# Fanchuana/OPUS-PLLM

Hardware: AMD Instinct MI355X
Metric: proteins_per_sec (higher is better)
Workload: dtype f16; 1 GPU; OPUS-PLLM-llama3_8b shape: batch 64/GPU, 512-residue proteins, 89-id prompt (+8 protein tokens = 96 positions), 32 new tokens, greedy (BASELINE configs[3] per-GPU shard: batch 512 over 8 GPUs); batch_per_gpu=64, residues=512, parallelism=replicas x1 (batch-sharded), all-gather of ids

## Files before the change

include/opus_pllm.h:

```cpp
#ifndef OPUS_PLLM_H
#define OPUS_PLLM_H

#include <stdint.h>

#ifdef __cplusplus
extern "C" {
#endif

#define OPUS_ABI_VERSION 10

enum opus_status {
    OPUS_OK = 0,
    OPUS_EBADARG = -1,
    OPUS_ESHAPE = -2,
    OPUS_EHIP = -3,
    OPUS_ERCCL = -4,
    OPUS_EUNSUPPORTED = -5,
    OPUS_ESTATE = -6
};

enum opus_dtype { OPUS_F16 = 0, OPUS_F32 = 1, OPUS_I32 = 2, OPUS_I64 = 3, OPUS_U8 = 4, OPUS_F8E4M3 = 5, OPUS_I8 = 6 };

typedef struct opus_config {
    int32_t enc_layers, enc_dim, enc_heads, enc_ffn, enc_vocab;
// ... 142 lines not shown
                                   int64_t n_slots, void *d_scratch, int64_t scratch_bytes, void *stream);

int opus_generate_lookup(opus_ctx *ctx, const void *d_embeds, const uint8_t *d_mask, int32_t B, int32_t T, int32_t max_new,
                         const int32_t *eos_ids, int32_t n_eos, int32_t pad_id, int32_t k, int32_t max_ngram, const int32_t *d_hist,
                         int32_t Lh, const int32_t *h_hist_len, int32_t *d_out_ids, int32_t *n_out, int64_t *stats, void *stream);
int opus_llama_verify_step(opus_ctx *ctx, const int32_t *d_tokens, int32_t n, const int32_t *d_draft_len, float *d_logits_all,
                           int32_t *d_argmax, int32_t *a, void *stream);
int opus_debug_lookup_draft(opus_ctx *ctx, const int32_t *d_hist, int32_t Lh, const int32_t *d_hist_len, int32_t R, int32_t k,
                            int32_t max_ngram, int32_t *d_draft, int32_t *d_draft_len, void *stream);
int opus_debug_last_qkv(opus_ctx *ctx, void *d_out, int32_t rows, void *stream);
int opus_debug_lookup_accept(opus_ctx *ctx, const int32_t *d_argmax, const int32_t *d_tokens, const int32_t *d_draft_len, int32_t R,
                             int32_t n, int32_t pre, int32_t *d_ids, int32_t stride, int32_t *d_fin, int32_t *d_step,
                             const int32_t *eos_ids, int32_t n_eos, int32_t pad_id, const int32_t *stop_ids, int32_t n_stop,
                             int32_t *d_next, int32_t *d_nunf, int32_t *h_words, void *stream);

int opus_debug_argmax_lse(opus_ctx *ctx, const float *d_logits, int32_t B, int32_t V, int32_t *d_idx, float *d_lse, void *stream);
int opus_debug_guidance(opus_ctx *ctx, float *d_logits, int32_t P, int32_t V, float guidance_scale, void *stream);

int opus_set_logits_processors(opus_ctx *ctx, float repetition_penalty, int32_t no_repeat_ngram_size, int32_t min_new_tokens,
                               const int32_t *bad_ids, const int32_t *bad_offsets, int32_t n_bad);
int opus_debug_logits_process(opus_ctx *ctx, float *d_logits, int32_t B, int32_t V, const int32_t *d_hist, int32_t hist_stride,
                              int32_t hist_len, const int32_t *eos_ids, int32_t n_eos, float repetition_penalty,
                              int32_t no_repeat_ngram_size, int32_t min_new_tokens, const int32_t *bad_ids,
                              const int32_t *bad_offsets, int32_t n_bad, void *stream);

int opus_set_token_constraint(opus_ctx *ctx, int32_t n_states, const int32_t *edge_off, const int32_t *edge_tok,
                              const int32_t *edge_next, int32_t n_edges, const uint8_t *completing, const int32_t *end_ids,
                              int32_t n_end, const int32_t *start, int32_t n_start, void *stream);
int opus_debug_token_constraint(opus_ctx *ctx, float *d_logits, int32_t B, int32_t V, const int32_t *d_hist, int32_t hist_stride,
                                int32_t hist_len, int32_t *d_state_out, void *stream);

int opus_debug_gemm(opus_ctx *ctx, const void *d_A, const void *d_W, const float *d_bias, const float *d_residual,
                    void *d_C, int32_t M, int32_t N, int32_t K, int32_t epi, int32_t out_f32, void *stream);
int opus_debug_gemm_norm(opus_ctx *ctx, const float *d_A, const void *d_W, void *d_C, int32_t M, int32_t N, int32_t K,
                         int32_t epi, int32_t out_f32, float eps, void *stream);
int opus_debug_gemm_slabs(opus_ctx *ctx, const void *d_A, const void *d_W, float *d_slabs, int32_t M, int32_t N, int32_t K,
                          int32_t *ks, void *stream);
int opus_debug_gemm_plan(opus_ctx *ctx, int32_t *plan);
int opus_debug_gemm_w8(opus_ctx *ctx, int32_t form, const void *d_A, const void *d_W, const void *d_q8, const void *d_e8,
                       const float *d_bias, const float *d_residual, void *d_C, int32_t M, int32_t N, int32_t K, int32_t epi,
                       int32_t out_f32, float eps, int32_t *ks, int32_t *ran_w8, void *stream);
int opus_debug_knob(opus_ctx *ctx, const char *name, int32_t value);
int opus_debug_gemm_rowscale(opus_ctx *ctx, const void *d_A, const void *d_W1, float *d_X, const void *d_W2, void *d_C,
                             int32_t M, int32_t N1, int32_t K1, int32_t N2, int32_t epi, float eps, int32_t *fused,
                             void *stream);
int opus_debug_gemm_rope(opus_ctx *ctx, const void *d_A, const void *d_W, const float *d_bias, void *d_out, int32_t M,
                         int32_t D, int32_t K, int32_t T, int32_t heads, int32_t allow_fuse, int32_t *fused, void *stream);
int opus_debug_gemm_ln(opus_ctx *ctx, const void *d_A, const void *d_W1, const float *d_b1, float *d_X, float *d_part, void *d_xh,
                       float *d_stat, const void *d_W2, const float *d_c2, const float *d_colsum, void *d_C, int32_t M, int32_t N1,
                       int32_t K1, int32_t N2, int32_t epi, int32_t rms, float eps, int32_t rope_T, const int32_t *d_rope_pos,
                       int32_t *produced, int32_t *plan, void *stream);
int opus_debug_attention(opus_ctx *ctx, const void *d_Q, const void *d_K, const void *d_V, void *d_O,
                         const int32_t *d_kstart, const int32_t *d_kend, int32_t B, int32_t T, int32_t heads,
                         int32_t group, int32_t head_dim, int32_t causal, float scale, void *stream);

int opus_debug_attn_prefill(opus_ctx *ctx, const void *d_Q, const void *d_K, const void *d_V, void *d_O, int64_t q_st, int64_t k_st,
                            int64_t v_st, int64_t o_st, int64_t q_sb, int64_t k_sb, int64_t v_sb, int64_t o_sb,
                            const int32_t *d_kstart, const int32_t *d_kend, const int32_t *d_cu, int32_t B, int32_t T,
                            int32_t heads, int32_t group, int32_t head_dim, int32_t causal, int32_t q_trim, float scale,
                            int32_t *qt_used, void *stream);

int opus_debug_attn_decode(opus_ctx *ctx, const void *d_qkv, const void *d_k_hist, const void *d_v_hist, const int32_t *d_kstart,
                           int32_t B, int32_t T0, int32_t step, void *d_out, void *d_k_new, void *d_v_new, void *stream);

int opus_debug_attn_decode_form(opus_ctx *ctx, const void *d_qkv, const float *d_slabs, int32_t ks, const float *d_row_ssq,
                                int32_t row_nblk, int32_t K, float eps, const float *d_bias, const void *d_k_hist,
                                const void *d_v_hist, const int32_t *d_kstart, int32_t B, int32_t T0, int32_t step,
                                int32_t out_tiled, void *d_out, void *d_k_new, void *d_v_new, void *d_k_cache, void *d_v_cache,
                                int32_t *gp_used, void *stream);

int opus_check_error(opus_ctx *ctx, void *stream);

int opus_beam_topk(opus_ctx *ctx, const float *d_run_scores, int32_t B, int32_t K, int32_t M, float *d_scores, int32_t *d_idx,
                   void *stream);
int opus_kv_reorder(opus_ctx *ctx, const int32_t *d_src_rows, int32_t R, void *stream);
int opus_beam_sample_topk(opus_ctx *ctx, const float *d_logits, const float *d_run_scores, int32_t B, int32_t K, int32_t M,
                          float temperature, float top_p, uint64_t seed, int32_t step, float *d_scores, int32_t *d_idx, void *stream);
int opus_set_sampling_top_k(opus_ctx *ctx, int32_t k);

int32_t opus_stream_lag(void);
int opus_stream_begin(opus_ctx *ctx, const void *d_embeds, const uint8_t *d_mask, int32_t B, int32_t T, int32_t max_new,
                      const int32_t *eos_ids, int32_t n_eos, int32_t pad_id, float temperature, float top_p, uint64_t seed,
                      int32_t *d_ids, void *stream);
int opus_stream_run(opus_ctx *ctx, int32_t t_min, int32_t min_free, int32_t t_max, int32_t *t_out, int32_t *h_end, void *stream);
int opus_stream_refill(opus_ctx *ctx, const opus_prefix_snap *snap, int32_t n, const int32_t *h_rows, const int32_t *h_src,
                       const float *d_last_logits, const int32_t *h_len, void *stream);
int opus_stream_end(opus_ctx *ctx, int32_t *h_end, void *stream);
int opus_debug_stream_state(opus_ctx *ctx, int32_t *h_kstart, int32_t *h_fin, int32_t *h_start, int32_t *h_end, int64_t *epoch,
                            int32_t poison, void *stream);

int opus_last_logits(opus_ctx *ctx, float *d_out, int32_t B, void *stream);

int64_t opus_stat(opus_ctx *ctx, const char *name);

int opus_timing_enable(opus_ctx *ctx, int32_t on);
int opus_timing_reset(opus_ctx *ctx);
int opus_timing_get(opus_ctx *ctx, const char *kernel_class, const char *phase, double *ms, int64_t *launches, double *bytes,
                    double *flops);
int opus_timing_names(char *buf, int32_t cap);

#ifdef __cplusplus
}
#endif
#endif
```

opus-pllm_amd/_cabi.py:

```python
from __future__ import annotations

import ctypes as C
import os
from typing import Optional

from .config import OpusConfig

_HERE = os.path.dirname(os.path.abspath(__file__))
BF16 = os.environ.get("OPUS_DTYPE", "fp16").lower() in ("bf16", "bfloat16")
LIB_PATH = os.environ.get("OPUS_LIB_PATH") or os.path.join(_HERE, "lib", "libopus_pllm_bf16.so" if BF16 else "libopus_pllm.so")
ABI_VERSION = 10

OPUS_F16, OPUS_F32, OPUS_I32, OPUS_I64, OPUS_U8 = 0, 1, 2, 3, 4
OPUS_F8E4M3, OPUS_I8 = 5, 6


def operand_dtype():
    import torch
    return torch.bfloat16 if BF16 else torch.float16


class OpusError(RuntimeError):
    def __init__(self, code: int, msg: str):
        super().__init__(f"libopus_pllm error {code}: {msg}")
# ... 65 lines not shown
    "opus_tile_weight": (C.c_int, [_P, _P, C.c_int64, C.c_int64, _P]),
    "opus_quantize_fp8": (C.c_int, [_P, C.c_int64, C.c_int64, _P, _P, _P, _P]),
    "opus_debug_gemm_w8": (C.c_int, [_P, C.c_int32, _P, _P, _P, _P, _P, _P, _P, C.c_int32, C.c_int32, C.c_int32, C.c_int32, C.c_int32,
                                     C.c_float, C.POINTER(C.c_int32), C.POINTER(C.c_int32), _P]),
    "opus_esm2_encode": (C.c_int, [_P, _P, _P, C.c_int32, C.c_int32, _P, _P]),
    "opus_esm2_encode_packed": (C.c_int, [_P, _P, C.POINTER(C.c_int32), C.c_int32, _P, _P]),
    "opus_esm2_last_hidden": (C.c_int, [_P, _P, C.c_int32, C.c_int32, _P]),
    "opus_projector_forward": (C.c_int, [_P, _P, C.c_int32, _P, _P, _P]),
    "opus_protein_projector": (C.c_int, [_P, _P, C.c_int32, _P, _P]),
    "opus_switch_projector": (C.c_int, [_P, _P, C.c_int32, _P, _P]),
    "opus_splice_pad": (C.c_int, [_P, _P, _P, C.c_int32, C.c_int32, _P, C.c_int32, C.c_int32, C.c_int32,
                                  _P, _P, _P, C.POINTER(C.c_int32), _P]),
    "opus_llama_prefill": (C.c_int, [_P, _P, _P, C.c_int32, C.c_int32, _P, _P]),
    "opus_llama_decode_step": (C.c_int, [_P, _P, _P, _P]),
    "opus_generate_greedy": (C.c_int, [_P, _P, _P, C.c_int32, C.c_int32, C.c_int32, C.POINTER(C.c_int32),
                                       C.c_int32, C.c_int32, _P, C.POINTER(C.c_int32), _P]),
    "opus_debug_gemm": (C.c_int, [_P, _P, _P, _P, _P, _P, C.c_int32, C.c_int32, C.c_int32, C.c_int32, C.c_int32, _P]),
    "opus_debug_gemm_norm": (C.c_int, [_P, _P, _P, _P, C.c_int32, C.c_int32, C.c_int32, C.c_int32, C.c_int32, C.c_float, _P]),
    "opus_debug_gemm_rope": (C.c_int, [_P, _P, _P, _P, _P, C.c_int32, C.c_int32, C.c_int32, C.c_int32, C.c_int32, C.c_int32, _P, _P]),
    "opus_debug_attention": (C.c_int, [_P, _P, _P, _P, _P, _P, _P, C.c_int32, C.c_int32, C.c_int32, C.c_int32,
                                       C.c_int32, C.c_int32, C.c_float, _P]),
    "opus_debug_attn_prefill": (C.c_int, [_P, _P, _P, _P, _P, C.c_int64, C.c_int64, C.c_int64, C.c_int64, C.c_int64, C.c_int64,
                                          C.c_int64, C.c_int64, _P, _P, _P, C.c_int32, C.c_int32, C.c_int32, C.c_int32, C.c_int32,
                                          C.c_int32, C.c_int32, C.c_float, C.POINTER(C.c_int32), _P]),
    "opus_generate_sample": (C.c_int, [_P, _P, _P, C.c_int32, C.c_int32, C.c_int32, C.POINTER(C.c_int32), C.c_int32, C.c_int32,
                                       C.c_float, C.c_float, C.c_uint64, _P, C.POINTER(C.c_int32), _P]),
    "opus_debug_sample": (C.c_int, [_P, _P, C.c_int32, C.c_float, C.c_float, C.c_uint64, C.c_int32, _P, _P]),
    "opus_timing_enable": (C.c_int, [_P, C.c_int32]),
    "opus_timing_reset": (C.c_int, [_P]),
    "opus_timing_get": (C.c_int, [_P, C.c_char_p, C.c_char_p, C.POINTER(C.c_double), C.POINTER(C.c_int64),
                                  C.POINTER(C.c_double), C.POINTER(C.c_double)]),
    "opus_timing_names": (C.c_int, [C.c_char_p, C.c_int32]),
    "opus_last_logits": (C.c_int, [_P, _P, C.c_int32, _P]),
    "opus_check_error": (C.c_int, [_P, _P]),
    "opus_beam_topk": (C.c_int, [_P, _P, C.c_int32, C.c_int32, C.c_int32, _P, _P, _P]),
    "opus_kv_reorder": (C.c_int, [_P, _P, C.c_int32, _P]),
    "opus_beam_sample_topk": (C.c_int, [_P, _P, _P, C.c_int32, C.c_int32, C.c_int32, C.c_float, C.c_float, C.c_uint64, C.c_int32,
                                        _P, _P, _P]),
    "opus_set_sampling_top_k": (C.c_int, [_P, C.c_int32]),
    "opus_set_stop_sequence": (C.c_int, [_P, C.POINTER(C.c_int32), C.c_int32]),
    "opus_debug_gemm_slabs": (C.c_int, [_P, _P, _P, _P, C.c_int32, C.c_int32, C.c_int32, C.POINTER(C.c_int32), _P]),
    "opus_debug_gemm_plan": (C.c_int, [_P, C.POINTER(C.c_int32)]),
    "opus_debug_knob": (C.c_int, [_P, C.c_char_p, C.c_int32]),
    "opus_stat": (C.c_int64, [_P, C.c_char_p]),
    "opus_debug_attn_decode": (C.c_int, [_P, _P, _P, _P, _P, C.c_int32, C.c_int32, C.c_int32, _P, _P, _P, _P]),
    "opus_debug_attn_decode_form": (C.c_int, [_P, _P, _P, C.c_int32, _P, C.c_int32, C.c_int32, C.c_float, _P, _P, _P, _P, C.c_int32,
                                              C.c_int32, C.c_int32, C.c_int32, _P, _P, _P, _P, _P, C.POINTER(C.c_int32), _P]),
    "opus_llama_forward": (C.c_int, [_P, _P, _P, C.c_int32, C.c_int32, _P, C.c_int32, _P, _P, _P, _P, C.c_int64, _P]),
    "opus_llama_forward_scratch_bytes": (C.c_int64, [C.POINTER(CConfig), C.c_int32, C.c_int32]),
    "opus_llama_prefix": (C.c_int, [_P, _P, _P, C.c_int32, C.c_int32, _P, _P, C.POINTER(C.c_int64), _P]),
    "opus_llama_score_continuations": (C.c_int, [_P, _P, C.c_int32, C.c_int32, _P, _P, _P, C.c_int32, C.c_int64, _P, _P, _P,
                                                 C.c_int64, _P]),
    "opus_llama_score_scratch_bytes": (C.c_int64, [C.POINTER(CConfig), C.c_int32, C.c_int32]),
    "opus_debug_attn_prefix": (C.c_int, [_P, _P, _P, _P, _P, C.c_int32, C.c_int32, C.c_int32, C.c_int32, _P, _P, _P]),
    "opus_llama_score_tree": (C.c_int, [_P, _P, C.c_int32, _P, _P, _P, C.c_int32, _P, C.c_int32, _P, _P, _P, C.c_int32, _P, _P, _P,
                                        C.c_int32, _P, C.c_int32, _P, _P, C.c_int32, C.c_int64, _P, _P, C.c_int64, _P, C.c_int64, _P]),
    "opus_llama_score_tree_scratch_bytes": (C.c_int64, [C.POINTER(CConfig), C.c_int32, C.c_int32, C.c_int32, C.c_int32, C.c_int32,
                                                        C.c_int32]),
    "opus_llama_dec_rows_cap": (C.c_int64, [C.POINTER(CConfig)]),
    "opus_llama_tree_max_depth": (C.c_int32, []),
    "opus_trie_path_sums": (C.c_int, [_P, _P, _P, _P, _P, _P, C.c_int32, C.c_int32, C.c_int32, _P, _P]),
    "opus_debug_attn_tree": (C.c_int, [_P, _P, _P, _P, _P, C.c_int32, C.c_int32, C.c_int32, _P, _P, _P, _P, _P]),
    "opus_debug_xent": (C.c_int, [_P, _P, C.c_int32, C.c_int32, _P, _P, _P, _P]),
    "opus_esm2_contacts_packed": (C.c_int, [_P, _P, C.POINTER(C.c_int32), C.c_int32, _P, _P, _P, C.c_int64, _P]),
    "opus_esm2_contacts_scratch_bytes": (C.c_int64, [C.POINTER(CConfig), C.POINTER(C.c_int32), C.c_int32]),
    "opus_debug_contacts": (C.c_int, [_P, _P, _P, C.c_int64, C.POINTER(C.c_int32), C.c_int32, C.c_int32, C.c_int32, _P, _P, _P, _P,
# ... 53 lines not shown
```

opus-pllm_amd/csrc/api.cpp:

```cpp
#include "../../include/opus_pllm.h"
#include "common.h"

#include <cmath>
#include <cstdarg>
#include <cstdio>
#include <cstdlib>
#include <cstring>
#include <algorithm>
#include <atomic>
#include <map>
#include <string>
#include <vector>

using namespace opus;

static thread_local char g_err[512] = "";
static int fail(int code, const char *fmt, ...) {
    va_list ap;
    va_start(ap, fmt);
    vsnprintf(g_err, sizeof(g_err), fmt, ap);
    va_end(ap);
    return code;
}
#define HIPC(expr)                                                                                   \
// ... 15 lines not shown
};

struct EncLayer {
    const float *bqkv, *bo, *b1, *b2, *sqkv, *s1;
    const half_t *wqkv, *wo, *w1, *w2;
};
struct DecLayer {
    const half_t *wqkv = nullptr, *wo = nullptr, *wgu = nullptr, *wd = nullptr;
    const float *bqkv = nullptr;
    const uint8_t *q8_qkv = nullptr, *q8_o = nullptr, *q8_gu = nullptr, *q8_d = nullptr;
    const int8_t *e8_qkv = nullptr, *e8_o = nullptr, *e8_gu = nullptr, *e8_d = nullptr;
    const half_t *w1 = nullptr, *w2 = nullptr;
    const float *bo = nullptr, *b1 = nullptr, *b2 = nullptr, *ln1w = nullptr, *ln1b = nullptr, *ln2w = nullptr, *ln2b = nullptr;
};

struct TimeRec {
    int klass, phase;
    hipEvent_t e0, e1;
    double bytes, flops;
};

struct StepPlan {
    int rows = -1;
    bool guided = false;
    int stride = -1;
    int32_t *ids = nullptr;
    int n_eos = -1, pad = 0;
    float temp = 0.f, top_p = 1.f;
    int top_k = 0, n_stop = 0;
    int outs = 0;
    bool lproc = false;
    bool cons = false;
    int budget = -1;
};
static bool same_step(const StepPlan &a, const StepPlan &b) {
    return a.rows == b.rows && a.guided == b.guided && a.stride == b.stride && a.ids == b.ids && a.n_eos == b.n_eos && a.pad == b.pad &&
           a.temp == b.temp && a.top_p == b.top_p && a.top_k == b.top_k && a.n_stop == b.n_stop && a.outs == b.outs &&
           a.lproc == b.lproc && a.cons == b.cons && a.budget == b.budget;
}

struct opus_ctx {
    opus_config cfg;
    int device = 0;
    std::map<std::string, Tensor> w;
    bool resolved = false;
    const half_t *enc_emb = nullptr, *dec_emb = nullptr, *lm_head = nullptr, *proj_w = nullptr, *dec_pos = nullptr;
    const float *enc_lnfw = nullptr, *enc_lnfb = nullptr, *proj_b = nullptr, *dec_lnfw = nullptr, *dec_lnfb = nullptr;
    std::vector<EncLayer> enc;
    std::vector<DecLayer> dec;
    std::vector<const half_t *> sw_w;
    std::vector<const float *> sw_b;
    char *ws = nullptr;
    size_t ws_bytes = 0;
    float *e_x, *e_hid, *p_pool_dummy, *e_part, *e_stat;
    int32_t *e_cu, *e_pos;
    std::vector<int32_t> h_cu;
    int64_t enc_rows = 0;
    half_t *e_xn, *e_qkv, *e_ctx, *e_h1;
    half_t *p_xn, *p_y, *p_z[2];
    float *d_x, *d_xl, *d_logits, *d_pval, *gemm_ws, *d_probs, *d_zpart, *d_spart, *d_part, *d_stat;
    int32_t *d_cand_i, *d_cand_n;
    uint64_t *d_seed;
    int32_t *d_chosen;
    int samp_top_k = 0;
    float *d_bthr = nullptr, *d_blse = nullptr;
    int64_t gemm_ws_bytes = 0;
    half_t *d_xn, *d_qkv, *d_ctx, *d_act, *d_xln, *kc, *vc;
    float *cs_enc, *cs_dec, *cs_row;
    int32_t *d_kstart, *d_step, *d_next, *d_fin, *d_nunf, *d_eos, *d_plan, *d_pidx, *d_stop, *d_cnt;
    int n_stop = 0;
    static constexpr int POLL_RING = 4, POLL_LAG = 2;
    int32_t *h_nunf = nullptr;
    hipEvent_t poll_ev[POLL_RING] = {nullptr, nullptr, nullptr, nullptr};
    int64_t cache_sl, cache_sb, cache_sh;
    int cur_B = 0, cur_T = 0;
    bool prefilled = false;
    struct GraphEntry {
        hipGraphExec_t exec = nullptr;
        StepPlan key;
        uint64_t used = 0;
    };
    static constexpr int MAX_GRAPHS = 4;
    std::vector<GraphEntry> graphs;
    uint64_t graph_clock = 0;
    int64_t graph_instantiations = 0;
    int64_t graph_replays = 0;
    int64_t decode_steps = 0;
    char *gen_mem = nullptr;
    GenOutDesc *d_gen = nullptr;
    GenOutDesc h_gen{};
    float *d_gpsum = nullptr, *d_gthr = nullptr;
    bool lproc_on = false;
    LogitsProcDesc h_lproc{1.0f, 0, 0, 0, {}, {}};
    char *lproc_mem = nullptr;
    LogitsProcDesc *d_lproc = nullptr;
    int32_t *d_lstep = nullptr, *d_ridx = nullptr;
    GenOutDesc *d_gen_raw = nullptr, *d_gen_proc = nullptr;
    float *d_rlse = nullptr, *d_rawh = nullptr;
    bool cons_on = false;
    char *cons_tab = nullptr, *cons_mem = nullptr;
    size_t cons_tab_bytes = 0;
    TokenConstraintDesc *d_cons = nullptr;
    int32_t *d_cstate = nullptr, *d_cstep = nullptr;
    int32_t cons_n_start = 0, cons_max_id = -1;
    int32_t cons_start_div = 1;
    char *guid_mem = nullptr;
    float *d_gscale = nullptr, *d_gdpsum = nullptr, *d_gmax = nullptr, *d_glog = nullptr, *d_glse = nullptr, *guid_keep = nullptr;
    int gemm_w8 = 0;
    int64_t w8_gemms = 0;
    int gemm_plan[GEMM_PLAN_WORDS] = {-1, -1, -1, -1, -1, -1, -1, -1};
    float *d_ssq = nullptr;
    int64_t ssq_cap = 0;
    bool timing = false;
    int phase = PH_OTHER;
    std::vector<TimeRec> recs;
    int proj_rows = 0;
    char *proj_big = nullptr;
    half_t *kv_tmp = nullptr;
    int64_t epoch = 0;
    std::vector<int32_t> h_kstart;
    int32_t *behind_tbl = nullptr;
// ... 210 lines not shown
    HIPC(hipMemset(c->kc, 0, (size_t)c->cache_sl * cfg->dec_layers * sizeof(half_t)));
    HIPC(hipMemset(c->vc, 0, (size_t)c->cache_sl * cfg->dec_layers * sizeof(half_t)));
    HIPC(hipHostMalloc((void **)&c->h_nunf, ((size_t)cfg->max_new_tokens + 4) * sizeof(int32_t), hipHostMallocDefault));
    for (auto &e : c->poll_ev) HIPC(hipEventCreateWithFlags(&e, hipEventDisableTiming));
    *out = c;
    return OPUS_OK;
}

static void timing_clear(opus_ctx *c) {
    for (auto &r : c->recs) {
        (void)hipEventDestroy(r.e0);
        (void)hipEventDestroy(r.e1);
    }
    c->recs.clear();
}

static void drop_graphs(opus_ctx *c) {
    for (auto &g : c->graphs)
        if (g.exec) (void)hipGraphExecDestroy(g.exec);
    c->graphs.clear();
    if (c->stream_graph.exec) (void)hipGraphExecDestroy(c->stream_graph.exec);
    c->stream_graph = opus_ctx::GraphEntry();
}

extern "C" int opus_ctx_destroy(opus_ctx *c) {
    if (!c) return OPUS_OK;
    (void)hipSetDevice(c->device);
    timing_clear(c);
    drop_graphs(c);
    if (c->ws) (void)hipFree(c->ws);
    if (c->proj_big) (void)hipFree(c->proj_big);
    if (c->kv_tmp) (void)hipFree(c->kv_tmp);
    if (c->gen_mem) (void)hipFree(c->gen_mem);
    if (c->lproc_mem) (void)hipFree(c->lproc_mem);
    if (c->cons_tab) (void)hipFree(c->cons_tab);
    if (c->cons_mem) (void)hipFree(c->cons_mem);
    if (c->guid_mem) (void)hipFree(c->guid_mem);
    if (c->guid_keep) (void)hipFree(c->guid_keep);
    if (c->behind_tbl) (void)hipFree(c->behind_tbl);
    if (c->h_nunf) (void)hipHostFree(c->h_nunf);
    if (c->stream_mem) (void)hipFree(c->stream_mem);
    if (c->h_poll) (void)hipHostFree(c->h_poll);
    if (c->lk_mem) (void)hipFree(c->lk_mem);
    if (c->h_lk) (void)hipHostFree(c->h_lk);
    for (auto &e : c->poll_ev) if (e) (void)hipEventDestroy(e);
    delete c;
    return OPUS_OK;
}

extern "C" int opus_bind_weight(opus_ctx *c, const char *name, const void *d_ptr, int dtype, int ndim,
                                const int64_t *shape) {
    if (!c || !name || !d_ptr || !shape) return fail(OPUS_EBADARG, "null argument");
    if (ndim < 1 || ndim > 4) return fail(OPUS_EBADARG, "ndim %d", ndim);
    const size_t nlen = strlen(name);
    const bool is_q8 = nlen > 3 && !strcmp(name + nlen - 3, ".q8"), is_e8 = nlen > 3 && !strcmp(name + nlen - 3, ".e8");
    if (is_q8 ? dtype != OPUS_F8E4M3 : is_e8 ? dtype != OPUS_I8 : (dtype != OPUS_F16 && dtype != OPUS_F32))
        return fail(OPUS_EBADARG, "weights are fp16 or fp32 (FP8 panels '*.q8': e4m3, their row exponents '*.e8': int8)");
    if (((uintptr_t)d_ptr) & 15) return fail(OPUS_EBADARG, "%s: pointer must be 16-byte aligned", name);
    Tensor t;
    t.p = d_ptr;
    t.dtype = dtype;
    t.shape.assign(shape, shape + ndim);
    c->w[name] = t;
    c->resolved = false;
    drop_graphs(c);
    return OPUS_OK;
// ... 119 lines not shown
        if (!c->timing) return;
        tl_launch_ev = nullptr;
        if (ev.main_used) {
            c->recs.push_back(TimeRec{ev.main_class >= 0 ? ev.main_class : klass, c->phase, ev.main0, ev.main1, bytes, flops});
            (void)hipEventDestroy(b0); (void)hipEventDestroy(b1);
        } else {
            (void)hipEventRecord(b1, s);
            c->recs.push_back(TimeRec{klass, c->phase, b0, b1, bytes, flops});
            (void)hipEventDestroy(ev.main0); (void)hipEventDestroy(ev.main1);
        }
        if (ev.aux_used) c->recs.push_back(TimeRec{KC_REDUCE, c->phase, ev.aux0, ev.aux1, ev.aux_bytes, 0.0});
        else { (void)hipEventDestroy(ev.aux0); (void)hipEventDestroy(ev.aux1); }
    }
};

struct GemmAsk {
    half_t *xh = nullptr;
    int xh_tiled = 0;
    bool rs_on = false;
    float rs_eps = 0.f;
    int rs_nblk = 0;
    const float *rope_cs = nullptr;
    const int32_t *rope_pos = nullptr;
    int rope_T = 0, rope_cols = 0, rope_qcols = 0;
    float rope_qscale = 1.0f;
    float *ln_part = nullptr;
    half_t *ln_xh = nullptr;
    const float *ln_stat = nullptr, *ln_colsum = nullptr;
    int force_wide = 0, slab_only = 0;
    int a_tiled = 0, c_tiled = 0;
    int *pp_plan = nullptr;
    const uint8_t *q8 = nullptr;
    const int8_t *e8 = nullptr;
    GemmAsk &copy16(half_t *dst, bool tiled = false) { xh = dst; xh_tiled = dst && tiled; return *this; }
    GemmAsk &scale_rows(float eps, int nblk) { rs_on = true; rs_eps = eps; rs_nblk = nblk; return *this; }
    GemmAsk &rope(const float *cs, const int32_t *pos, int T, int D, float qscale) {
        if (cs) { rope_cs = cs; rope_pos = pos; rope_T = T; rope_cols = 2 * D; rope_qcols = D; rope_qscale = qscale; }
        return *this;
    }
    GemmAsk &ln_produce(float *part, half_t *x16) { if (part) { ln_part = part; ln_xh = x16; } return *this; }
    GemmAsk &ln_consume(const float *stat, const float *colsum) { if (stat) { ln_stat = stat; ln_colsum = colsum; } return *this; }
    GemmAsk &slabs() { force_wide = slab_only = 1; return *this; }
    GemmAsk &tiled_a(int on) { a_tiled = on; return *this; }
    GemmAsk &tiled_c(int on) { c_tiled = on; return *this; }
    GemmAsk &report_pp(int *plan) { pp_plan = plan; return *this; }
    GemmAsk &w8(const uint8_t *q, const int8_t *e) { if (q && e) { q8 = q; e8 = e; } return *this; }
};
struct GemmGot {
    int xh_done = 0, rope_done = 0, ln_done = 0, ks = 1, ssq_nblk = 0;
};

static int gemm_any(opus_ctx *c, hipStream_t s, const half_t *A, const float *Af, float eps, int64_t lda, const half_t *W,
                    int M, int N, int K, const float *bias, int epi, const float *residual, void *C, int64_t ldc,
                    int out_f32, const GemmAsk &ask = GemmAsk(), GemmGot *got = nullptr) {
    GemmGot mine;
    if (!got) got = &mine;
    *got = GemmGot();
    GemmParams p;
    p.A = A; p.Af = Af; p.norm_eps = eps; p.lda = lda; p.W = W; p.M = M; p.N = N; p.K = K; p.bias = bias;
    p.residual = residual; p.ldr = ldc; p.C = C; p.ldc = ldc; p.out_f32 = out_f32; p.epi = epi;
    p.ws = c->gemm_ws; p.ws_bytes = c->gemm_ws_bytes;
    p.xh_out = ask.xh; p.ssq_out = c->d_ssq; p.fused_done = &got->xh_done; p.ssq_cap = c->ssq_cap; p.nblk_out = &got->ssq_nblk;
    p.rope_cs = ask.rope_cs; p.rope_T = ask.rope_T; p.rope_cols = ask.rope_cols; p.rope_qcols = ask.rope_qcols;
    p.rope_qscale = ask.rope_qscale; p.rope_done = &got->rope_done; p.rope_pos = ask.rope_pos;
    p.row_ssq = nullptr; p.row_nblk = 0;
    if (ask.rs_on) { p.row_ssq = c->d_ssq; p.row_nblk = ask.rs_nblk; p.norm_eps = ask.rs_eps; }
    p.force_wide = ask.force_wide; p.slab_only = ask.slab_only; p.ks_out = &got->ks;
    if (ask.ln_part) { p.xh_out = ask.ln_xh; p.ssq_out = nullptr; p.ln_part = ask.ln_part; p.ln_done = &got->ln_done; }
    if (ask.ln_stat) { p.ln_stat = ask.ln_stat; p.ln_colsum = ask.ln_colsum; }
    p.combine_cnt = c->d_cnt;
    p.pp_plan = ask.pp_plan;
    for (int i = 0; i < GEMM_PLAN_WORDS; ++i) c->gemm_plan[i] = -1;
    p.plan = c->gemm_plan;
    c->gemm_w8 = 0;
    p.q8 = ask.q8; p.e8 = ask.e8; p.ran_w8 = &c->gemm_w8;
    p.a_tiled = ask.a_tiled; p.xh_tiled = ask.xh_tiled; p.c_tiled = ask.c_tiled;
    const int nout = epi == EPI_SILU_GU16 ? N / 2 : N;
    const double bytes = 2.0 * N * K + (Af ? 4.0 : 2.0) * M * K + (double)M * nout * (out_f32 ? 4 : 2) +
                         (residual ? 4.0 * M * nout : 0.0);
    int klass = M <= SKINNY_MAX_M ? KC_SKINNY : KC_TILE;
    hipError_t e;
    {
        Timed t(c, s, klass, bytes, 2.0 * M * N * (double)K);
        e = launch_gemm(p, s, &klass);
    }
    if (e != hipSuccess) return fail(OPUS_EHIP, "gemm M=%d N=%d K=%d failed: %s", M, N, K, hipGetErrorString(e));
    c->w8_gemms += c->gemm_w8;
    return OPUS_OK;
}
static int gemm(opus_ctx *c, hipStream_t s, const half_t *A, int64_t lda, const half_t *W, int M, int N, int K,
                const float *bias, int epi, const float *residual, void *C, int64_t ldc, int out_f32,
                const GemmAsk &ask = GemmAsk(), GemmGot *got = nullptr) {
    return gemm_any(c, s, A, nullptr, 0.f, lda, W, M, N, K, bias, epi, residual, C, ldc, out_f32, ask, got);
}
struct ResidShadow {
    const float *xh_src = nullptr;
    int ssq_nblk = 0;
    bool xln_tiled = false;
    void produced(const float *x, const GemmGot &got, bool tiled = false) {
        xh_src = got.xh_done ? x : nullptr;
        if (got.xh_done) ssq_nblk = got.ssq_nblk;
        xln_tiled = got.xh_done && tiled;
    }
};
static bool fuse_rows() {
    static const bool off = getenv("OPUS_NO_ROW_FUSION") != nullptr;
    return !off;
}
#define KLF(klass, bytes, flops, call)                                                                \
    do {                                                                                              \
        hipError_t e_;                                                                                \
        {                                                                                             \
            Timed t_(c, s, klass, bytes, flops);                                                      \
            e_ = (call);                                                                              \
        }                                                                                             \
        if (e_ != hipSuccess) return fail(OPUS_EHIP, "%s failed: %s", #call, hipGetErrorString(e_)); \
    } while (0)
#define KL(klass, bytes, call) KLF(klass, bytes, 0.0, call)

// ... 435 lines not shown
        const int n = B - r0 < c->proj_rows ? B - r0 : c->proj_rows;
        OPC(protein_projector_rows(c, s, d_pooled + r0 * din, n, c->p_y));
        if (d_proj_out)
            HIPC(hipMemcpyAsync((half_t *)d_proj_out + r0 * dmid, c->p_y, (size_t)n * dmid * sizeof(half_t), hipMemcpyDeviceToDevice, s));
        OPC(switch_projector_rows(c, s, c->p_y, n, (half_t *)d_out + r0 * SW));
    }
    return OPUS_OK;
}

extern "C" int opus_splice_pad(opus_ctx *c, const int64_t *d_ids, const uint8_t *d_mask, int32_t B, int32_t Tt,
                               const void *d_prot, int32_t n_prot, int32_t inference_mode, int32_t max_length,
                               void *d_embeds, uint8_t *d_mask_out, int32_t *d_pos_out, int32_t *T_out, void *stream) {
    OPC(need_ready(c));
    if (!d_ids || !d_prot || !d_embeds || !d_mask_out || !d_pos_out || !T_out) return fail(OPUS_EBADARG, "splice_pad: null pointer");
    const opus_config &g = c->cfg;
    if (B < 1 || B > g.max_batch || Tt < 1) return fail(OPUS_ESHAPE, "splice_pad: B=%d T_text=%d out of range", B, Tt);
    hipStream_t s = (hipStream_t)stream;
    c->phase = PH_SPLICE;
    KL(KC_OTHER, 9.0 * B * Tt, launch_splice_plan(d_ids, d_mask, B, Tt, g.n_prot_tokens, max_length, g.dec_vocab, c->d_plan, s));
    int32_t tail[3];
    HIPC(hipMemcpyAsync(tail, c->d_plan + 4 * B, sizeof(tail), hipMemcpyDeviceToHost, s));
    HIPC(hipStreamSynchronize(s));
    if (tail[2]) return fail(OPUS_EBADARG, "splice_pad: token id outside [0, vocab) (and not -200)");
    if (tail[1] > n_prot) return fail(OPUS_ESHAPE, "splice_pad: rows consume %d protein blocks, %d supplied", tail[1], n_prot);
    if (tail[0] > g.max_prompt) return fail(OPUS_ESHAPE, "splice_pad: spliced length %d exceeds max_prompt=%d", tail[0], g.max_prompt);
    if (tail[0] < 1) return fail(OPUS_ESHAPE, "splice_pad: every row is empty");
    *T_out = tail[0];
    KL(KC_OTHER, 2.0 * B * tail[0] * g.dec_dim * 2,
       launch_splice_fill(d_ids, d_mask, B, Tt, (const half_t *)d_prot, g.n_prot_tokens, g.dec_dim, g.dec_vocab, c->dec_emb,
                          c->d_plan, tail[0], inference_mode ? 1 : 0, (half_t *)d_embeds, d_mask_out, d_pos_out, s));
    return OPUS_OK;
}

static int lm_head(opus_ctx *c, hipStream_t s, ResidShadow &sh, int B, float *out = nullptr) {
    const opus_config &g = c->cfg;
    return gemm_norm(c, s, sh, c->d_xl, g.dec_rms_eps, c->d_xln, c->lm_head, B, g.dec_vocab, g.dec_dim, EPI_NONE, out ? out : c->d_logits,
                     g.dec_vocab, 1);
}

static int fanout_rows(opus_ctx *c, hipStream_t s, int B, int nret) {
    const opus_config &g = c->cfg;
    KL(KC_OTHER, 4.0 * (B + B * nret) * g.dec_vocab, launch_row_fanout(c->d_probs, c->d_logits, g.dec_vocab, B, nret, c->d_kstart, s));
    return OPUS_OK;
}


static int reset_step(opus_ctx *c, hipStream_t s, int T0, int step = 0) {
    const int32_t v[2] = {step, T0};
    HIPC(launch_upload_i32(v, 2, c->d_step, s));
    return OPUS_OK;
}

template <class Head>
static int finish_prefill(opus_ctx *c, hipStream_t s, int B, int T, int nret, bool have_last, Head head) {
    const int H = c->cfg.dec_dim;
    if (!have_last) KL(KC_OTHER, 8.0 * B * H, launch_take_last(c->d_x, B, T, H, c->d_xl, s));
    OPC(head(nret > 1 ? c->d_probs : nullptr));
    if (nret > 1) OPC(fanout_rows(c, s, B, nret));
    OPC(reset_step(c, s, T));
    c->cur_B = B * nret;
    c->cur_T = T;
    c->prefilled = true;
    return OPUS_OK;
}

static int attn_decode(opus_ctx *c, hipStream_t s, const ResidShadow &sh, int l, int B, int T, int slab_ks = 0, const float *bias = nullptr,
                       int out_tiled = 0) {
    const opus_config &g = c->cfg;
    AttnDecodeParams a;
    a.qkv = c->d_qkv; a.slabs = nullptr; a.ks = 0; a.slab_stride = 0; a.row_ssq = nullptr; a.row_nblk = 0; a.eps = 0.f; a.K = 0;
// ... 41 lines not shown
    a.q_sb = a.k_sb = a.v_sb = (int64_t)T * QKV;
    a.q_st = a.k_st = a.v_st = QKV;
    a.O = c->d_ctx; a.o_sb = (int64_t)T * QD; a.o_st = QD;
    a.kstart = c->d_kstart; a.kend = nullptr;
    a.B = B; a.T = T; a.heads = nh; a.group = nh / nkv; a.head_dim = hd; a.causal = 1;
    a.scale = 1.0f / sqrtf((float)hd);
    KLF(KC_ATTN_PREFILL, 2.0 * M * (QKV + QD), 2.0 * B * (double)T * T * QD, launch_attn_prefill(a, s));
    return OPUS_OK;
}

static int opt_layer(opus_ctx *c, hipStream_t s, const DecLayer &L, int l, float *x, half_t *xn, int M, int B, int T, bool decode,
                     const ContRows *cont = nullptr, int nret = 1) {
    const opus_config &g = c->cfg;
    const int H = g.dec_dim, F = g.dec_ffn;
    const int QKV = (g.dec_heads + 2 * g.dec_kv_heads) * g.dec_head_dim, QD = g.dec_heads * g.dec_head_dim;
    KL(KC_NORM, 6.0 * M * H, launch_layernorm(x, L.ln1w, L.ln1b, g.dec_rms_eps, M, H, xn, nullptr, s));
    OPC(gemm(c, s, xn, H, L.wqkv, M, QKV, H, L.bqkv, EPI_NONE, nullptr, c->d_qkv, QKV, 0));
    if (decode) OPC(attn_decode(c, s, ResidShadow(), l, B, T));
    else OPC(attn_prefill(c, s, l, B, T, cont, nret));
    OPC(gemm(c, s, c->d_ctx, QD, L.wo, M, H, QD, L.bo, EPI_NONE, x, x, H, 1));
    KL(KC_NORM, 6.0 * M * H, launch_layernorm(x, L.ln2w, L.ln2b, g.dec_rms_eps, M, H, xn, nullptr, s));
    if (g.dec_act == 0) {
        OPC(gemm(c, s, xn, H, L.w1, M, F, H, L.b1, EPI_GELU, nullptr, c->d_act, F, 0));
    } else {
        OPC(gemm(c, s, xn, H, L.w1, M, F, H, L.b1, EPI_NONE, nullptr, c->d_act, F, 0));
        KL(KC_OTHER, 4.0 * M * F, launch_relu_h(c->d_act, (int64_t)M * F, s));
    }
    OPC(gemm(c, s, c->d_act, F, L.w2, M, H, F, L.b2, EPI_NONE, x, x, H, 1));
    return OPUS_OK;
}

static int lm_head_opt(opus_ctx *c, hipStream_t s, int B, float *out = nullptr) {
    const opus_config &g = c->cfg;
    KL(KC_NORM, 6.0 * B * g.dec_dim, launch_layernorm(c->d_xl, c->dec_lnfw, c->dec_lnfb, g.dec_rms_eps, B, g.dec_dim, c->d_xln, nullptr, s));
    return gemm(c, s, c->d_xln, g.dec_dim, c->lm_head, B, g.dec_vocab, g.dec_dim, nullptr, EPI_NONE, nullptr, out ? out : c->d_logits,
                g.dec_vocab, 1);
}

static int prefill_opt(opus_ctx *c, hipStream_t s, const half_t *embeds, const uint8_t *mask, int B, int T, bool all_rows,
                       const ContRows *cont, int nret) {
    const opus_config &g = c->cfg;
    const int H = g.dec_dim, M = B * T;
    HIPC(hipMemsetAsync(c->d_cnt, 0, HANDOFF_ERR * sizeof(int32_t), s));
    if (!cont) KL(KC_OTHER, 1.0 * M, launch_mask_to_kstart(mask, B, T, c->d_kstart, s));
    KL(KC_OTHER, 6.0 * M * H, launch_h2f(embeds, c->d_x, (int64_t)M * H, s));
    KL(KC_OTHER, 10.0 * M * H, launch_add_pos(c->d_x, c->dec_pos, cont ? cont->nkst : c->d_kstart, nullptr, 0, B, T, H, g.dec_max_pos + 1, s));
    for (int l = 0; l < g.dec_layers; ++l) OPC(opt_layer(c, s, c->dec[l], l, c->d_x, c->d_xn, M, B, T, false, cont, nret));
    if (all_rows) return OPUS_OK;
    return finish_prefill(c, s, B, T, nret, false, [&](float *out) { return lm_head_opt(c, s, B, out); });
}

static int decode_step_opt(opus_ctx *c, hipStream_t s) {
    const opus_config &g = c->cfg;
    const int B = c->cur_B, T = c->cur_T, H = g.dec_dim;
    KL(KC_OTHER, 10.0 * B * H, launch_add_pos(c->d_xl, c->dec_pos, c->d_kstart, c->d_step, -1, B, 1, H, g.dec_max_pos + 1, s));
    for (int l = 0; l < g.dec_layers; ++l) OPC(opt_layer(c, s, c->dec[l], l, c->d_xl, c->d_xln, B, B, T, true));
    OPC(lm_head_opt(c, s, B));
    KL(KC_OTHER, 8.0, launch_step_advance(c->d_step, s));
    return OPUS_OK;
}

static int prefill(opus_ctx *c, hipStream_t s, const half_t *embeds, const uint8_t *mask, int B, int T, bool all_rows = false,
                   const ContRows *cont = nullptr, int nret = 1) {
    c->phase = cont && !cont->app_lens ? PH_SCORE : PH_PREFILL;
    if (cont && cont->w8) c->phase = PH_DECODE;
    if (cont) {
        all_rows = true;
    } else {
        new_epoch(c);
        if (all_rows) {
            c->prefilled = false;
            c->cur_B = 0;
        }
    }
    if (c->cfg.dec_arch == 1) return prefill_opt(c, s, embeds, mask, B, T, all_rows, cont, nret);
    const opus_config &g = c->cfg;
    const int H = g.dec_dim, F = g.dec_ffn, nh = g.dec_heads, nkv = g.dec_kv_heads, hd = g.dec_head_dim;
    const int QKV = (nh + 2 * nkv) * hd, QD = nh * hd;
    const int M = B * T;
    HIPC(hipMemsetAsync(c->d_cnt, 0, HANDOFF_ERR * sizeof(int32_t), s));
    if (!cont) KL(KC_OTHER, 1.0 * M, launch_mask_to_kstart(mask, B, T, c->d_kstart, s));
    KL(KC_OTHER, 6.0 * M * H, launch_h2f(embeds, c->d_x, (int64_t)M * H, s));
    static const bool no_ln_env = getenv("OPUS_NO_LN_FUSION") != nullptr;
    const bool no_ln_fusion = no_ln_env || g_knobs.no_ln_fusion;
    const bool qkv_pp = !no_ln_fusion && (H & 255) == 0 && (QKV & 255) == 0 && gemm_goes_pp(M, QKV);
    const bool gu_pp = !no_ln_fusion && (H & 255) == 0 && (F & 127) == 0 && gemm_goes_pp(M, 2 * F);
    bool have_stat = false, last_rows_done = false;
    auto finalize = [&]() -> int {
        KL(KC_NORM, 8.0 * M * (H / 64) + 8.0 * M, launch_ln_finalize(c->d_part, M, H / 64, H, g.dec_rms_eps, 1, c->d_stat, s));
        return OPUS_OK;
    };
    ResidShadow sh;
    GemmGot got;
    const bool w8 = cont && cont->w8;
    auto ask8 = [&](GemmAsk a, const uint8_t *q, const int8_t *e) { return w8 ? a.w8(q, e) : a; };
    for (int l = 0; l < g.dec_layers; ++l) {
// ... 7 lines not shown
        OPC(attn_prefill(c, s, l, B, T, cont, nret));
        if (l + 1 == g.dec_layers && T > 1 && !all_rows && !g_knobs.misc[7]) {
            half_t *ctx_last = c->d_qkv;
            KL(KC_OTHER, 4.0 * B * QD, launch_take_last(reinterpret_cast<const float *>(c->d_ctx), B, T, QD / 2, reinterpret_cast<float *>(ctx_last), s));
            KL(KC_OTHER, 8.0 * B * H, launch_take_last(c->d_x, B, T, H, c->d_xl, s));
            const GemmAsk copy_xl = GemmAsk().copy16(fuse_rows() && B <= 96 ? c->d_xln : nullptr);
            OPC(gemm(c, s, ctx_last, QD, L.wo, B, H, QD, nullptr, EPI_NONE, c->d_xl, c->d_xl, H, 1, copy_xl, &got));
            sh.produced(c->d_xl, got);
            OPC(gemm_norm(c, s, sh, c->d_xl, g.dec_rms_eps, c->d_xln, L.wgu, B, 2 * F, H, EPI_SILU_GU16, c->d_act, F, 0));
            OPC(gemm(c, s, c->d_act, F, L.wd, B, H, F, nullptr, EPI_NONE, c->d_xl, c->d_xl, H, 1, copy_xl, &got));
            sh.produced(c->d_xl, got);
            last_rows_done = true;
            break;
        }
        GemmAsk wo;
        if (gu_pp) wo.ln_produce(c->d_part, c->d_xn);
        else if (fuse_rows() && M <= 96) wo.copy16(c->d_xn);
        OPC(gemm(c, s, c->d_ctx, QD, L.wo, M, H, QD, nullptr, EPI_NONE, c->d_x, c->d_x, H, 1, ask8(wo, L.q8_o, L.e8_o), &got));
        sh.produced(c->d_x, got);
        have_stat = got.ln_done != 0;
        if (have_stat) {
            OPC(finalize());
            OPC(gemm(c, s, c->d_xn, H, L.wgu, M, 2 * F, H, nullptr, EPI_SILU_GU16, nullptr, c->d_act, F, 0, GemmAsk().ln_consume(c->d_stat, nullptr)));
        } else {
            OPC(gemm_norm(c, s, sh, c->d_x, g.dec_rms_eps, c->d_xn, L.wgu, M, 2 * F, H, EPI_SILU_GU16, c->d_act, F, 0, nullptr,
                          ask8(GemmAsk(), L.q8_gu, L.e8_gu)));
        }
        const bool next_pp = qkv_pp && l + 1 < g.dec_layers;
        OPC(gemm(c, s, c->d_act, F, L.wd, M, H, F, nullptr, EPI_NONE, c->d_x, c->d_x, H, 1, ask8(GemmAsk().ln_produce(next_pp ? c->d_part : nullptr, c->d_xn), L.q8_d, L.e8_d), &got));
        have_stat = got.ln_done != 0;
        if (have_stat) OPC(finalize());
    }
    if (all_rows) return OPUS_OK;
    return finish_prefill(c, s, B, T, nret, last_rows_done, [&](float *out) { return lm_head(c, s, sh, B, out); });
}

static int decode_step(opus_ctx *c, hipStream_t s, const int32_t *d_tok) {
    c->phase = PH_DECODE;
    const opus_config &g = c->cfg;
    const int B = c->cur_B, T = c->cur_T;
    const int H = g.dec_dim, F = g.dec_ffn, nh = g.dec_heads, nkv = g.dec_kv_heads, hd = g.dec_head_dim;
    const int QKV = (nh + 2 * nkv) * hd, QD = nh * hd;
    const int ctx_cap = g.max_prompt + g.max_new_tokens;
    const bool rowscale = g.dec_arch == 0 && fuse_rows() && B > SKINNY_MAX_M && B <= MID_MAX_M && (H & 255) == 0;
    const bool qkv_tiled = rowscale && gemm_stream_would(B, QKV, H, 1, 1, 1, c->gemm_ws_bytes);
    const bool wo_tiled = rowscale && gemm_stream_would(B, H, QD, 0, 1, 0, c->gemm_ws_bytes);
    const bool down_tiled = rowscale && (F & 63) == 0 && gemm_stream_would(B, H, F, 0, 1, 0, c->gemm_ws_bytes);
    KL(KC_OTHER, 6.0 * B * H, launch_embed_tokens(d_tok, c->dec_emb, B, H, g.dec_vocab, c->d_xl, rowscale ? c->d_xln : nullptr,
                                                  rowscale ? c->d_ssq : nullptr, qkv_tiled ? 1 : 0, c->cs_dec, c->d_kstart, c->d_step, -1,
                                                  hd / 2, c->cs_row, c->d_cnt, HANDOFF_ERR, s));
    if (g.dec_arch == 1) return decode_step_opt(c, s);
    ResidShadow sh;
    if (rowscale) { sh.xh_src = c->d_xl; sh.ssq_nblk = H >> 8; sh.xln_tiled = qkv_tiled; }
    GemmGot got;
    half_t *const copy_xl = fuse_rows() && B <= 96 ? c->d_xln : nullptr;
    for (int l = 0; l < g.dec_layers; ++l) {
        const DecLayer &L = c->dec[l];
        if (rowscale && sh.xh_src == c->d_xl) {
            sh.xh_src = nullptr;
            OPC(gemm(c, s, c->d_xln, H, L.wqkv, B, QKV, H, L.bqkv, EPI_NONE, nullptr, c->d_qkv, QKV, 0,
                     GemmAsk().slabs().scale_rows(g.dec_rms_eps, sh.ssq_nblk).tiled_a(sh.xln_tiled).w8(L.q8_qkv, L.e8_qkv), &got));
            OPC(attn_decode(c, s, sh, l, B, T, got.ks > 1 ? got.ks : 0, L.bqkv, wo_tiled ? 1 : 0));
        } else {
            OPC(gemm_norm(c, s, sh, c->d_xl, g.dec_rms_eps, c->d_xln, L.wqkv, B, QKV, H, EPI_NONE, c->d_qkv, QKV, 0, L.bqkv,
                          GemmAsk().w8(L.q8_qkv, L.e8_qkv)));
            OPC(attn_decode(c, s, sh, l, B, T, 0, nullptr, wo_tiled ? 1 : 0));
        }
        OPC(gemm(c, s, c->d_ctx, QD, L.wo, B, H, QD, nullptr, EPI_NONE, c->d_xl, c->d_xl, H, 1, GemmAsk().copy16(copy_xl).tiled_a(wo_tiled).w8(L.q8_o, L.e8_o), &got));
        sh.produced(c->d_xl, got);
        const bool act_tiled = down_tiled && sh.xh_src == c->d_xl && gemm_goes_wide(B, 2 * F);
        OPC(gemm_norm(c, s, sh, c->d_xl, g.dec_rms_eps, c->d_xln, L.wgu, B, 2 * F, H, EPI_SILU_GU16, c->d_act, F, 0, nullptr, GemmAsk().tiled_c(act_tiled).w8(L.q8_gu, L.e8_gu)));
        const bool next_tiled = qkv_tiled && l + 1 < g.dec_layers;
        OPC(gemm(c, s, c->d_act, F, L.wd, B, H, F, nullptr, EPI_NONE, c->d_xl, c->d_xl, H, 1, GemmAsk().copy16(copy_xl, next_tiled).tiled_a(act_tiled).w8(L.q8_d, L.e8_d), &got));
        sh.produced(c->d_xl, got, next_tiled);
    }
    OPC(lm_head(c, s, sh, B));
    KL(KC_OTHER, 8.0, launch_step_advance(c->d_step, s));
    return OPUS_OK;
}

static int handoff_check(opus_ctx *c, hipStream_t s) {
    int32_t err = 0;
    HIPC(hipMemcpyAsync(&err, c->d_cnt + HANDOFF_ERR, sizeof(err), hipMemcpyDeviceToHost, s));
    HIPC(hipStreamSynchronize(s));
    if (!err) return OPUS_OK;
    HIPC(hipMemsetAsync(c->d_cnt, 0, HANDOFF_WORDS * sizeof(int32_t), s));
    return fail(OPUS_EHIP, "an in-launch hand-off (split-K combine) gave up waiting for its partner: results of this call are invalid");
}

extern "C" int opus_check_error(opus_ctx *c, void *stream) {
    if (!c) return fail(OPUS_EBADARG, "ctx is null");
    HIPC(hipSetDevice(c->device));
    return handoff_check(c, (hipStream_t)stream);
}

static int check_prefill_args(opus_ctx *c, const void *e, const uint8_t *m, int B, int T) {
    if (!e || !m) return fail(OPUS_EBADARG, "prefill: null pointer");
    if (B < 1 || B > c->cfg.max_batch || T < 1 || T > c->cfg.max_prompt)
        return fail(OPUS_ESHAPE, "prefill: B=%d T=%d exceed capacity (%d, %d)", B, T, c->cfg.max_batch, c->cfg.max_prompt);
    return OPUS_OK;
}

extern "C" int opus_llama_prefill(opus_ctx *c, const void *d_embeds, const uint8_t *d_mask, int32_t B, int32_t T,
                                  float *d_last_logits, void *stream) {
    OPC(need_ready(c));
    OPC(check_prefill_args(c, d_embeds, d_mask, B, T));
    hipStream_t s = (hipStream_t)stream;
    OPC(prefill(c, s, (const half_t *)d_embeds, d_mask, B, T));
    if (d_last_logits)
// ... 693 lines not shown
    if (P < 1 || M < 1 || ld_nodes < 2) return fail(OPUS_ESHAPE, "trie_path_sums: P=%d M=%d nodes=%d", P, M, ld_nodes);
    HIPC(hipSetDevice(c->device));
    hipStream_t s = (hipStream_t)stream;
    c->phase = PH_SCORE;
    KL(KC_OTHER, 12.0 * P * M, launch_tree_path_sums(d_node_lp, d_trie, d_par, d_depth, d_member_node, P, M, ld_nodes, d_member_lp, s));
    return OPUS_OK;
}

extern "C" int opus_debug_attn_tree(opus_ctx *c, const void *d_qkv, const void *d_k_hist, const void *d_v_hist, const int32_t *d_kstart,
                                    int32_t P, int32_t Tp, int32_t R, const int32_t *h_src, const int32_t *h_par, const int32_t *h_depth,
                                    void *d_out, void *stream) {
    if (!c || !d_qkv || !d_k_hist || !d_v_hist || !d_kstart || !h_src || !h_par || !h_depth || !d_out)
        return fail(OPUS_EBADARG, "debug_attn_tree: null pointer");
    const opus_config &g = c->cfg;
    if (P < 1 || P > g.max_batch || Tp < 1 || Tp > g.max_prompt || R < 1)
        return fail(OPUS_ESHAPE, "debug_attn_tree: P=%d Tp=%d R=%d exceed the context (%d, %d)", P, Tp, R, g.max_batch, g.max_prompt);
    OPC(check_tree_rows("debug_attn_tree", R, P, h_src, h_par, h_depth));
    return debug_attn_prefix_run(c, "debug_attn_tree", d_qkv, d_k_hist, d_v_hist, d_kstart, P, Tp, R, 1, h_src, h_par, d_out, stream);
}

enum { GEN_LOGPROBS = 1, GEN_SCORES = 2, GEN_LOGITS = 4 };

static int ensure_gen_mem(opus_ctx *c) {
    if (c->gen_mem) return OPUS_OK;
    const size_t B = c->cfg.max_batch;
    const size_t o_ps = align_up(sizeof(GenOutDesc)), o_thr = o_ps + align_up(APART * B * sizeof(float));
    HIPC(hipMalloc((void **)&c->gen_mem, o_thr + align_up(B * sizeof(float))));
    c->d_gen = reinterpret_cast<GenOutDesc *>(c->gen_mem);
    c->d_gpsum = reinterpret_cast<float *>(c->gen_mem + o_ps);
    c->d_gthr = reinterpret_cast<float *>(c->gen_mem + o_thr);
    return OPUS_OK;
}

static int ensure_lproc_mem(opus_ctx *c) {
    if (c->lproc_mem) return OPUS_OK;
    const size_t B = c->cfg.max_batch, N = c->cfg.max_new_tokens;
    const size_t o_st = align_up(sizeof(LogitsProcDesc)), o_gr = o_st + align_up(B * sizeof(int32_t)),
                 o_gp = o_gr + align_up(sizeof(GenOutDesc)), o_ls = o_gp + align_up(sizeof(GenOutDesc)),
                 o_rh = o_ls + align_up(B * sizeof(float));
    HIPC(hipMalloc((void **)&c->lproc_mem, o_rh + align_up(B * N * sizeof(float))));
    c->d_lproc = reinterpret_cast<LogitsProcDesc *>(c->lproc_mem);
    c->d_ridx = reinterpret_cast<int32_t *>(c->lproc_mem + o_st);
    c->d_lstep = c->d_ridx;
    c->d_gen_raw = reinterpret_cast<GenOutDesc *>(c->lproc_mem + o_gr);
    c->d_gen_proc = reinterpret_cast<GenOutDesc *>(c->lproc_mem + o_gp);
    c->d_rlse = reinterpret_cast<float *>(c->lproc_mem + o_ls);
    c->d_rawh = reinterpret_cast<float *>(c->lproc_mem + o_rh);
    return OPUS_OK;
}

static int ensure_guid_mem(opus_ctx *c, bool keep) {
    const size_t B = c->cfg.max_batch;
    if (!c->guid_mem) {
        const size_t rows = align_up(2 * B * sizeof(float));
        const size_t o_ps = align_up(sizeof(float)), o_mx = o_ps + align_up(APART * B * sizeof(float)), o_lg = o_mx + rows,
                     o_ls = o_lg + rows;
        HIPC(hipMalloc((void **)&c->guid_mem, o_ls + rows));
        c->d_gscale = reinterpret_cast<float *>(c->guid_mem);
        c->d_gdpsum = reinterpret_cast<float *>(c->guid_mem + o_ps);
        c->d_gmax = reinterpret_cast<float *>(c->guid_mem + o_mx);
        c->d_glog = reinterpret_cast<float *>(c->guid_mem + o_lg);
        c->d_glse = reinterpret_cast<float *>(c->guid_mem + o_ls);
    }
    if (keep && !c->guid_keep) HIPC(hipMalloc((void **)&c->guid_keep, align_up((B / 2) * (size_t)c->cfg.dec_vocab * sizeof(float))));
    return OPUS_OK;
}
// ... 3 lines not shown
    memcpy(&w, &g, sizeof(w));
    HIPC(launch_upload_i32(&w, 1, reinterpret_cast<int32_t *>(c->d_gscale), s));
    return OPUS_OK;
}

static int upload_lproc(opus_ctx *c, const LogitsProcDesc &h, hipStream_t s) {
    const int32_t *w = reinterpret_cast<const int32_t *>(&h);
    const int head = (int)(offsetof(LogitsProcDesc, bad_off) / sizeof(int32_t)) + h.n_bad + 1;
    int32_t *dw = reinterpret_cast<int32_t *>(c->d_lproc);
    HIPC(launch_upload_i32(w, head, dw, s));
    const int n_ids = h.bad_off[h.n_bad];
    const int o_ids = (int)(offsetof(LogitsProcDesc, bad_ids) / sizeof(int32_t));
    if (n_ids) HIPC(launch_upload_i32(w + o_ids, n_ids, dw + o_ids, s));
    return OPUS_OK;
}

static int upload_gen_desc(const GenOutDesc &h, GenOutDesc *d, hipStream_t s) {
    HIPC(launch_upload_i32(reinterpret_cast<const int32_t *>(&h), (int)(sizeof(GenOutDesc) / sizeof(int32_t)),
                           reinterpret_cast<int32_t *>(d), s));
    return OPUS_OK;
}

static int select_next(opus_ctx *c, hipStream_t s, const StepPlan &p) {
    const int max_new = p.stride, n_eos = p.n_eos, pad_id = p.pad;
    int32_t *d_out = p.ids;
    c->phase = PH_DECODE;
    const opus_config &g = c->cfg;
    const int32_t *chosen = nullptr;
    const bool guid = p.guided;
    const int HB = guid ? p.rows / 2 : p.rows;
    const bool proc = p.lproc || p.cons || guid;
    const bool lp = p.outs & GEN_LOGPROBS, sc = p.outs & (GEN_SCORES | GEN_LOGITS);
    const size_t BV = (size_t)HB * g.dec_vocab;
    if (proc) {
        if (p.outs & GEN_LOGITS)
            KL(KC_OTHER, 8.0 * BV, launch_gen_scores(c->d_logits, HB, g.dec_vocab, c->d_gen_raw, c->d_step, max_new, 0.f, 1.f,
                                                     nullptr, nullptr, s));
        if (guid) {
            KL(KC_GUIDANCE, 8.0 * BV, launch_guidance_lse_partial(c->d_logits, 2 * HB, g.dec_vocab, c->d_pval, c->d_gdpsum, s));
            KL(KC_GUIDANCE, 1024.0 * HB, launch_guidance_lse_final(c->d_pval, c->d_gdpsum, 2 * HB, c->d_gmax, c->d_glog, c->d_glse, s));
            KL(KC_GUIDANCE, (lp ? 16.0 : 12.0) * BV,
               launch_guidance_combine(c->d_logits, c->d_logits + BV, HB, g.dec_vocab, c->d_gmax, c->d_glog, c->d_gmax + HB,
                                       c->d_glog + HB, c->d_gscale, lp ? c->guid_keep : nullptr, s));
        } else if (lp) {
            KL(KC_OTHER, 4.0 * BV, launch_argmax_lse_partial(c->d_logits, HB, g.dec_vocab, c->d_pval, c->d_pidx, c->d_gpsum, s));
            KL(KC_OTHER, 512.0 * HB, launch_argmax_lse_final(c->d_pval, c->d_pidx, c->d_gpsum, HB, c->d_ridx, c->d_rlse, s));
        }
        if (p.lproc)
            KL(KC_LOGITPROC, 12.0 * HB * max_new,
               launch_logits_proc(c->d_logits, HB, g.dec_vocab, d_out, max_new, c->d_step, max_new, c->d_eos, n_eos, c->d_lproc,
                                  lp && !guid ? c->d_rawh : nullptr, s));
        if (p.cons)
            KL(KC_CONSTRAINT, 4.0 * BV,
               launch_token_constraint(c->d_logits, HB, g.dec_vocab, d_out, max_new, c->d_step, max_new, c->d_cons, s));
    }
    if (p.temp > 0.f) {
        KL(KC_OTHER, 4.0 * 4 * HB * g.dec_vocab,
           launch_sample_select(c->d_logits, HB, g.dec_vocab, p.temp, p.top_p, p.top_k, c->d_seed, c->d_step,
                                c->d_pval, c->d_pidx, c->d_probs, c->d_cand_i, c->d_cand_n, c->d_zpart, c->d_spart, c->d_chosen, nullptr,
                                lp && !proc ? c->d_gpsum : nullptr, sc ? c->d_gthr : nullptr, s));
        chosen = c->d_chosen;
    } else if (lp && !proc) {
        KL(KC_OTHER, 4.0 * HB * g.dec_vocab,
           launch_argmax_lse_partial(c->d_logits, HB, g.dec_vocab, c->d_pval, c->d_pidx, c->d_gpsum, s));
    } else {
        KL(KC_OTHER, 4.0 * HB * g.dec_vocab, launch_argmax_partial(c->d_logits, HB, g.dec_vocab, c->d_pval, c->d_pidx, s));
    }
    if (proc ? (p.outs & GEN_SCORES) != 0 : sc)
        KL(KC_OTHER, 4.0 * HB * g.dec_vocab * (1 + ((p.outs & GEN_SCORES) ? 1 : 0) + ((p.outs & GEN_LOGITS) && !proc ? 1 : 0)),
           launch_gen_scores(c->d_logits, HB, g.dec_vocab, proc ? c->d_gen_proc : c->d_gen, c->d_step, max_new, p.temp,
                             p.top_p, c->d_pval, p.temp > 0.f ? c->d_gthr : nullptr, s));
    if (lp && proc)
        KL(KC_OTHER, 512.0 * HB + 8.0 * HB * max_new,
           launch_argmax_rawlp_step(c->d_pval, c->d_pidx, guid ? c->d_glse : c->d_rlse, p.lproc && !guid ? c->d_rawh : nullptr, chosen, HB, c->d_eos, n_eos, pad_id, c->d_fin, d_out,
                                    max_new, c->d_step, c->d_next, c->d_nunf, c->d_stop, p.n_stop, guid ? c->guid_keep : c->d_logits,
                                    g.dec_vocab, c->d_gen_proc, s));
    else if (lp)
        KL(KC_OTHER, 512.0 * HB + 8.0 * HB,
           launch_argmax_lse_step(c->d_pval, c->d_pidx, c->d_gpsum, chosen, HB, c->d_eos, n_eos, pad_id, c->d_fin, d_out, max_new,
                                  c->d_step, c->d_next, c->d_nunf, c->d_stop, p.n_stop, c->d_logits, g.dec_vocab, c->d_gen, s));
    else
        KL(KC_OTHER, 512.0 * HB,
           launch_argmax_step(c->d_pval, c->d_pidx, chosen, HB, c->d_eos, n_eos, pad_id, c->d_fin, d_out, max_new, c->d_step,
                              c->d_next, c->d_nunf, c->d_stop, p.n_stop, s));
    if (guid) KL(KC_GUIDANCE, 8.0 * HB, launch_guidance_pair_next(c->d_next, HB, s));
    return OPUS_OK;
}

static int greedy_body(opus_ctx *c, hipStream_t s, const StepPlan &p) {
    OPC(select_next(c, s, p));
    return decode_step(c, s, c->d_next);
}

static int capture_step(opus_ctx *c, hipStream_t s, int (*body)(opus_ctx *, hipStream_t, const StepPlan &), const StepPlan &p,
                        hipGraphExec_t *exec) {
    hipGraph_t graph = nullptr;
    HIPC(hipStreamBeginCapture(s, hipStreamCaptureModeThreadLocal));
    int rc = body(c, s, p);
    hipError_t ee = hipStreamEndCapture(s, &graph);
    if (rc != OPUS_OK) { if (graph) (void)hipGraphDestroy(graph); return rc; }
    if (ee != hipSuccess) return fail(OPUS_EHIP, "hipStreamEndCapture: %s", hipGetErrorString(ee));
    ee = hipGraphInstantiate(exec, graph, nullptr, nullptr, 0);
    (void)hipGraphDestroy(graph);
    if (ee != hipSuccess) { *exec = nullptr; return fail(OPUS_EHIP, "hipGraphInstantiate: %s", hipGetErrorString(ee)); }
    ++c->graph_instantiations;
    return OPUS_OK;
}

static int begin_generation(opus_ctx *c, const char *who, float temperature, float top_p, int32_t max_new, const int32_t *eos_ids,
                            int32_t n_eos, const uint64_t *seed, int rows, int steps, hipStream_t s) {
    if (temperature < 0.f || top_p <= 0.f || top_p > 1.f) return fail(OPUS_EBADARG, "%s: temperature >= 0 and 0 < top_p <= 1", who);
    if (max_new < 1 || max_new > c->cfg.max_new_tokens)
        return fail(OPUS_ESHAPE, "%s: max_new=%d exceeds max_new_tokens=%d", who, max_new, c->cfg.max_new_tokens);
    if (n_eos < 0 || n_eos > 64 || (n_eos > 0 && !eos_ids)) return fail(OPUS_EBADARG, "%s: eos list", who);
    if (n_eos) HIPC(hipMemcpyAsync(c->d_eos, eos_ids, n_eos * sizeof(int32_t), hipMemcpyHostToDevice, s));
    HIPC(hipMemcpyAsync(c->d_seed, seed, sizeof(*seed), hipMemcpyHostToDevice, s));
    HIPC(hipMemsetAsync(c->d_fin, 0, rows * sizeof(int32_t), s));
    HIPC(hipMemsetAsync(c->d_nunf, 0, (size_t)steps * sizeof(int32_t), s));
    return OPUS_OK;
}

static int set_cons_start_div(opus_ctx *c, int32_t div, hipStream_t s) {
    if (div == c->cons_start_div) return OPUS_OK;
    int32_t *w = reinterpret_cast<int32_t *>(c->d_cons) + offsetof(TokenConstraintDesc, start_div) / sizeof(int32_t);
    HIPC(launch_upload_i32(&div, 1, w, s));
    c->cons_start_div = div;
    return OPUS_OK;
}

static int generate_impl(opus_ctx *c, const void *d_embeds, const uint8_t *d_mask, int32_t B, int32_t T, int32_t max_new,
                         const int32_t *eos_ids, int32_t n_eos, int32_t pad_id, float temperature, float top_p, uint64_t seed,
                         int32_t *d_out_ids, int32_t *n_out, void *stream, const GenOutDesc *outs = nullptr, int32_t nret = 1,
                         const BehindArgs *behind = nullptr, const float *guidance = nullptr) {
    OPC(need_ready(c));
    if (!behind) OPC(check_prefill_args(c, d_embeds, d_mask, B, T));
    else if (B < 1 || B > c->cfg.max_batch) return fail(OPUS_ESHAPE, "generate: B=%d decoder rows, the context holds max_batch=%d", B, c->cfg.max_batch);
    OPC(check_fanout(c, B, nret, "generate"));
    const int32_t BN = B * nret;
    if (!d_out_ids || !n_out) return fail(OPUS_EBADARG, "generate_greedy: null pointer");
    hipStream_t s = (hipStream_t)stream;
    const opus_config &g = c->cfg;
    OPC(begin_generation(c, "generate_greedy", temperature, top_p, max_new, eos_ids, n_eos, &seed, BN, max_new, s));
    StepPlan plan;
    plan.rows = BN; plan.guided = guidance != nullptr; plan.stride = max_new; plan.ids = d_out_ids; plan.n_eos = n_eos; plan.pad = pad_id;
    plan.temp = temperature; plan.top_p = top_p; plan.top_k = c->samp_top_k; plan.n_stop = c->n_stop;
    plan.lproc = c->lproc_on; plan.cons = c->cons_on;
    if (outs) plan.outs = (outs->token_lp ? GEN_LOGPROBS : 0) | (outs->scores ? GEN_SCORES : 0) | (outs->logits ? GEN_LOGITS : 0);
    if (plan.outs) {
        OPC(ensure_gen_mem(c));
        c->h_gen = *outs;
        HIPC(hipMemcpyAsync(c->d_gen, &c->h_gen, sizeof(GenOutDesc), hipMemcpyHostToDevice, s));
    }
    const int32_t HB = guidance ? B / 2 : B;
    if (c->cons_on && c->cons_n_start != 1 && c->cons_n_start != HB)
        return fail(OPUS_ESHAPE, "generate: the token constraint has %d per-row start states, the batch %d rows", c->cons_n_start, HB);
    if (c->cons_on) OPC(set_cons_start_div(c, nret, s));
    if (guidance) {
        OPC(ensure_guid_mem(c, plan.outs & GEN_LOGPROBS));
        OPC(upload_guidance_scale(c, *guidance, s));
    }
    if (c->lproc_on || c->cons_on || guidance) {
        if (c->lproc_on && max_new > LP_MAX_HIST)
            return fail(OPUS_ESHAPE, "generate: logits processors keep a history of at most %d ids (max_new=%d)", LP_MAX_HIST, max_new);
        OPC(ensure_lproc_mem(c));
        if (c->lproc_on) OPC(upload_lproc(c, c->h_lproc, s));
        if (plan.outs) {
            OPC(upload_gen_desc(GenOutDesc{nullptr, nullptr, outs->logits, nullptr}, c->d_gen_raw, s));
            OPC(upload_gen_desc(GenOutDesc{outs->token_lp, outs->scores, nullptr, nullptr}, c->d_gen_proc, s));
        }
    }
    if (behind) OPC(prefill_behind(c, s, *behind, (const half_t *)d_embeds, B, T));
    else OPC(prefill(c, s, (const half_t *)d_embeds, d_mask, B, T, false, nullptr, nret));

    const bool use_graph = s != nullptr && !c->timing && !getenv("OPUS_NO_GRAPH");
    opus_ctx::GraphEntry *ge = nullptr;
    if (use_graph)
        for (auto &e : c->graphs)
            if (e.exec && same_step(e.key, plan)) { ge = &e; break; }
    const bool same_graph = ge != nullptr;
    std::vector<int32_t> nunf(max_new, 1);
    int produced = 0;
    for (int i = 0; i < max_new; ++i) {
        if (i + 1 == max_new) {
            OPC(select_next(c, s, plan));
            produced = i + 1;
            break;
        }
        ++c->decode_steps;
        if (!use_graph || (i == 0 && !same_graph)) {
            OPC(greedy_body(c, s, plan));
        } else {
            if (!ge) {
                opus_ctx::GraphEntry e;
                OPC(capture_step(c, s, greedy_body, plan, &e.exec));
                e.key = plan;
                if ((int)c->graphs.size() >= opus_ctx::MAX_GRAPHS) {
                    size_t v = 0;
                    for (size_t k = 1; k < c->graphs.size(); ++k) if (c->graphs[k].used < c->graphs[v].used) v = k;
                    (void)hipGraphExecDestroy(c->graphs[v].exec);
                    c->graphs.erase(c->graphs.begin() + v);
                }
                c->graphs.push_back(e);
                ge = &c->graphs.back();
            }
            ge->used = ++c->graph_clock;
// ... 499 lines not shown
    c->lk_kstart.assign((size_t)c->cur_B, 0);
    HIPC(hipMemcpyAsync(c->lk_kstart.data(), c->d_kstart, (size_t)c->cur_B * sizeof(int32_t), hipMemcpyDeviceToHost, s));
    HIPC(hipStreamSynchronize(s));
    c->lk_epoch = c->epoch;
    return OPUS_OK;
}

static int verify_pass(opus_ctx *c, hipStream_t s, const int32_t *x, int ld_x, int n, int Tp) {
    const opus_config &g = c->cfg;
    const int R = c->cur_B, M = R * n, H = g.dec_dim, V = g.dec_vocab, G = g.dec_heads / g.dec_kv_heads;
    if (!c->behind_tbl) HIPC(hipMalloc((void **)&c->behind_tbl, (size_t)behind_table_words(g) * sizeof(int32_t)));
    std::vector<int32_t> src((size_t)R);
    for (int r = 0; r < R; ++r) src[r] = r;
    PrefixTables t;
    build_prefix_tables(g, c->lk_kstart, Tp, src.data(), R, n, t);
    if (t.nblocks > attn_prefix_max_blocks(R, g.max_batch, G, n)) return fail(OPUS_EHIP, "verify pass: block table overflow");
    const int o_lens = (int)t.w.size();
    t.w.insert(t.w.end(), (size_t)R, n);
    if ((int64_t)t.w.size() > behind_table_words(g)) return fail(OPUS_EHIP, "verify pass: table overflow");
    int32_t *tbl = c->behind_tbl;
    c->phase = PH_DECODE;
    HIPC(launch_upload_i32(t.w.data(), (int)t.w.size(), tbl, s));
    KL(KC_OTHER, 4.0 * M * H, launch_lookup_embed(x, ld_x, R, n, c->dec_emb, H, V, c->d_xn, s));
    ContRows cr;
    cr.nkst = tbl + t.nkst;
    cr.nblocks = t.nblocks;
    cr.attn = prefix_params(c, tbl, t, Tp, n, c->d_qkv, nullptr, nullptr, c->d_ctx);
    cr.app_lens = tbl + o_lens;
    cr.w8 = true;
    OPC(prefill(c, s, c->d_xn, nullptr, R, n, true, &cr));
    c->phase = PH_DECODE;
    if (g.dec_arch == 1) {
        KL(KC_NORM, 6.0 * M * H, launch_layernorm(c->d_x, c->dec_lnfw, c->dec_lnfb, g.dec_rms_eps, M, H, c->d_xn, nullptr, s));
        OPC(gemm(c, s, c->d_xn, H, c->lm_head, M, V, H, nullptr, EPI_NONE, nullptr, c->d_logits, V, 1));
    } else {
        ResidShadow none;
        OPC(gemm_norm(c, s, none, c->d_x, g.dec_rms_eps, c->d_xn, c->lm_head, M, V, H, EPI_NONE, c->d_logits, V, 1));
    }
    ++c->lookup_passes;
    return OPUS_OK;
}

static int lookup_argmax(opus_ctx *c, hipStream_t s, int rows, int32_t *out) {
    const int V = c->cfg.dec_vocab;
    KL(KC_OTHER, 4.0 * rows * V, launch_argmax_partial(c->d_logits, rows, V, c->d_pval, c->d_pidx, s));
    KL(KC_OTHER, 512.0 * rows, launch_lookup_argmax(c->d_pval, c->d_pidx, rows, out, s));
    return OPUS_OK;
}

static int lookup_words(opus_ctx *c, hipStream_t s, int nwords) {
    HIPC(hipMemcpyAsync(c->h_lk, c->d_lk_words, (size_t)nwords * sizeof(int32_t), hipMemcpyDeviceToHost, s));
    HIPC(hipStreamSynchronize(s));
    return OPUS_OK;
}

static int check_lookup_state(opus_ctx *c, const char *who) {
    if (!c->prefilled) return fail(OPUS_ESTATE, "%s before prefill", who);
    if (c->st.on) return fail(OPUS_ESTATE, "%s: a continuous session is open on this context", who);
    if (c->cur_B > 64) return fail(OPUS_ESHAPE, "%s: %d decoder rows (at most 64)", who, c->cur_B);
    return OPUS_OK;
}

extern "C" int opus_llama_verify_step(opus_ctx *c, const int32_t *d_tokens, int32_t n, const int32_t *d_draft_len, float *d_logits_all,
                                      int32_t *d_argmax, int32_t *a, void *stream) {
    OPC(need_ready(c));
    OPC(check_lookup_state(c, "verify_step"));
    if (!d_tokens || !a) return fail(OPUS_EBADARG, "verify_step: null pointer");
    const opus_config &g = c->cfg;
    const int R = c->cur_B;
// ... 147 lines not shown
    OPC(ensure_gen_mem(c));
    hipStream_t s = (hipStream_t)stream;
    c->phase = PH_OTHER;
    KL(KC_OTHER, 4.0 * B * V, launch_argmax_lse_partial(d_logits, B, V, c->d_pval, c->d_pidx, c->d_gpsum, s));
    KL(KC_OTHER, 512.0 * B, launch_argmax_lse_final(c->d_pval, c->d_pidx, c->d_gpsum, B, d_idx, d_lse, s));
    return OPUS_OK;
}

extern "C" int opus_debug_sample(opus_ctx *c, const float *d_logits, int32_t B, float temperature, float top_p, uint64_t seed,
                                 int32_t step, int32_t *d_tokens, void *stream) {
    if (!c || !d_logits || !d_tokens) return fail(OPUS_EBADARG, "debug_sample: null pointer");
    if (B < 1 || B > c->cfg.max_batch || !(temperature > 0.f) || top_p <= 0.f || top_p > 1.f) return fail(OPUS_EBADARG, "debug_sample: argument");
    HIPC(hipSetDevice(c->device));
    hipStream_t s = (hipStream_t)stream;
    HIPC(hipMemcpyAsync(c->d_seed, &seed, sizeof(seed), hipMemcpyHostToDevice, s));
    HIPC(hipMemcpyAsync(c->d_plan, &step, sizeof(step), hipMemcpyHostToDevice, s));
    HIPC(launch_sample_select(d_logits, B, c->cfg.dec_vocab, temperature, top_p, c->samp_top_k, c->d_seed, c->d_plan, c->d_pval, c->d_pidx,
                              c->d_probs, c->d_cand_i, c->d_cand_n, c->d_zpart, c->d_spart, d_tokens, nullptr, nullptr, nullptr, s));
    HIPC(hipStreamSynchronize(s));
    return OPUS_OK;
}

extern "C" int opus_debug_gemm(opus_ctx *c, const void *A, const void *W, const float *bias, const float *residual,
                               void *Cp, int32_t M, int32_t N, int32_t K, int32_t epi, int32_t out_f32, void *stream) {
    if (!c || !A || !W || !Cp) return fail(OPUS_EBADARG, "debug_gemm: null pointer");
    if (M < 1 || N < 1 || K < 64 || K % 64) return fail(OPUS_ESHAPE, "debug_gemm: K must be a positive multiple of 64");
    if (epi < 0 || epi > 2 || (epi == 2 && N % 32)) return fail(OPUS_EBADARG, "debug_gemm: epilogue");
    HIPC(hipSetDevice(c->device));
    const int nout = epi == EPI_SILU_GU16 ? N / 2 : N;
    return gemm(c, (hipStream_t)stream, (const half_t *)A, K, (const half_t *)W, M, N, K, bias, epi, residual, Cp, nout,
                out_f32, GemmAsk().tiled_a(g_knobs.debug_a_tiled));
}

extern "C" int opus_debug_gemm_norm(opus_ctx *c, const float *A, const void *W, void *Cp, int32_t M, int32_t N, int32_t K,
                                    int32_t epi, int32_t out_f32, float eps, void *stream) {
    if (!c || !A || !W || !Cp) return fail(OPUS_EBADARG, "debug_gemm_norm: null pointer");
    if (M < 1 || M > MID_MAX_M || N < 1 || K < 64 || K % 64) return fail(OPUS_ESHAPE, "debug_gemm_norm: M <= 64, K %% 64 == 0");
    if (epi != 0 && epi != 2) return fail(OPUS_EBADARG, "debug_gemm_norm: epilogue 0 or 2");
    HIPC(hipSetDevice(c->device));
    const int nout = epi == EPI_SILU_GU16 ? N / 2 : N;
    return gemm_any(c, (hipStream_t)stream, nullptr, A, eps, K, (const half_t *)W, M, N, K, nullptr, epi, nullptr, Cp, nout,
                    out_f32);
}

extern "C" int opus_debug_gemm_rope(opus_ctx *c, const void *A, const void *W, const float *bias, void *out, int32_t M,
                                    int32_t D, int32_t K, int32_t T, int32_t heads, int32_t allow_fuse, int32_t *fused,
                                    void *stream) {
    if (!c || !A || !W || !out || !fused) return fail(OPUS_EBADARG, "debug_gemm_rope: null pointer");
    if (M < 1 || D < 16 || K < 64 || K % 64 || T < 1 || heads < 1 || D % heads || M % T)
        return fail(OPUS_ESHAPE, "debug_gemm_rope: M %% T == 0, D %% heads == 0, K %% 64 == 0");
    const int hd = D / heads;
    if (hd != c->cfg.enc_dim / c->cfg.enc_heads || T > c->cfg.max_enc_tokens)
        return fail(OPUS_ESHAPE, "debug_gemm_rope: head_dim / T must match the context's encoder rotary table");
    HIPC(hipSetDevice(c->device));
    hipStream_t s = (hipStream_t)stream;
    const float qs = 1.0f / sqrtf((float)hd);
    GemmGot got;
    OPC(gemm(c, s, (const half_t *)A, K, (const half_t *)W, M, 3 * D, K, bias, EPI_NONE, nullptr, out, 3 * D, 0,
             GemmAsk().rope(allow_fuse && hd == 64 ? c->cs_enc : nullptr, nullptr, T, D, qs), &got));
    *fused = got.rope_done;
    if (!got.rope_done) HIPC(launch_esm_rope((half_t *)out, c->cs_enc, M / T, T, heads, hd, qs, s));
    return OPUS_OK;
}

extern "C" int opus_debug_gemm_rowscale(opus_ctx *c, const void *A, const void *W1, float *X, const void *W2, void *Cp, int32_t M,
                                        int32_t N1, int32_t K1, int32_t N2, int32_t epi, float eps, int32_t *fused, void *stream) {
// ... 146 lines not shown
       launch_beam_sample(lg, d_run_scores, B, K, V, M, temperature, c->d_pval, c->d_bthr, min_keep, c->d_probs, c->d_cand_i, seed, step,
                          c->d_blse, d_scores, d_idx, s));
    return OPUS_OK;
}

extern "C" int opus_set_sampling_top_k(opus_ctx *c, int32_t k) {
    if (!c || k < 0) return fail(OPUS_EBADARG, "set_sampling_top_k: k >= 0");
    if (k != c->samp_top_k) drop_graphs(c);
    c->samp_top_k = k;
    return OPUS_OK;
}

extern "C" int opus_kv_reorder(opus_ctx *c, const int32_t *d_src_rows, int32_t R, void *stream) {
    if (!c || !d_src_rows) return fail(OPUS_EBADARG, "kv_reorder: null pointer");
    if (!c->prefilled || R != c->cur_B) return fail(OPUS_ESHAPE, "kv_reorder: R=%d but the last prefill had %d rows", R, c->prefilled ? c->cur_B : 0);
    HIPC(hipSetDevice(c->device));
    hipStream_t s = (hipStream_t)stream;
    const opus_config &g = c->cfg;
    const size_t row = (size_t)c->cache_sb, layer = row * g.max_batch;
    if (!c->kv_tmp) HIPC(hipMalloc((void **)&c->kv_tmp, 2 * layer * sizeof(half_t)));
    c->phase = PH_DECODE;
    new_epoch(c);
    const int nkv = g.dec_kv_heads, hd = g.dec_head_dim, T0 = c->cur_T;
    for (int l = 0; l < g.dec_layers; ++l) {
        half_t *kc = c->kc + l * c->cache_sl, *vc = c->vc + l * c->cache_sl;
        KL(KC_OTHER, 8.0 * R * nkv * hd * T0, launch_kv_gather_rows(kc, c->kv_tmp, d_src_rows, R, (int64_t)row, nkv, c->cache_sh, c->d_step, T0, hd, 0, s));
        HIPC(launch_kv_gather_rows(vc, c->kv_tmp + layer, d_src_rows, R, (int64_t)row, nkv, c->cache_sh, c->d_step, T0, hd, 0, s));
        HIPC(launch_kv_gather_rows(kc, c->kv_tmp, d_src_rows, R, (int64_t)row, nkv, c->cache_sh, c->d_step, T0, hd, 1, s));
        HIPC(launch_kv_gather_rows(vc, c->kv_tmp + layer, d_src_rows, R, (int64_t)row, nkv, c->cache_sh, c->d_step, T0, hd, 1, s));
    }
    return OPUS_OK;
}

extern "C" int opus_last_logits(opus_ctx *c, float *d_out, int32_t B, void *stream) {
    if (!c || !d_out) return fail(OPUS_EBADARG, "last_logits: null pointer");
    if (!c->prefilled) return fail(OPUS_ESTATE, "last_logits before prefill");
    if (B < 1 || B > c->cur_B) return fail(OPUS_ESHAPE, "last_logits: B=%d but the last prefill had %d rows", B, c->cur_B);
    HIPC(hipSetDevice(c->device));
    HIPC(hipMemcpyAsync(d_out, c->d_logits, (size_t)B * c->cfg.dec_vocab * sizeof(float), hipMemcpyDeviceToDevice, (hipStream_t)stream));
    return OPUS_OK;
}

extern "C" int opus_debug_attention(opus_ctx *c, const void *Q, const void *K, const void *V, void *O,
                                    const int32_t *kstart, const int32_t *kend, int32_t B, int32_t T, int32_t heads,
                                    int32_t group, int32_t hd, int32_t causal, float scale, void *stream) {
    if (!c || !Q || !K || !V || !O) return fail(OPUS_EBADARG, "debug_attention: null pointer");
    if (B < 1 || T < 1 || heads < 1 || group < 1 || heads % group) return fail(OPUS_ESHAPE, "debug_attention: shape");
    HIPC(hipSetDevice(c->device));
    hipStream_t s = (hipStream_t)stream;
    AttnParams a;
    const int kvh = heads / group;
    a.Q = (const half_t *)Q; a.K = (const half_t *)K; a.V = (const half_t *)V; a.O = (half_t *)O;
    a.q_st = (int64_t)heads * hd; a.q_sb = a.q_st * T;
    a.k_st = a.v_st = (int64_t)kvh * hd; a.k_sb = a.v_sb = a.k_st * T;
    a.o_st = a.q_st; a.o_sb = a.q_sb;
    a.kstart = kstart; a.kend = kend; a.B = B; a.T = T; a.heads = heads; a.group = group; a.head_dim = hd;
    a.causal = causal; a.scale = scale;
    KLF(KC_ATTN_PREFILL, 2.0 * B * T * hd * (2.0 * heads + 2.0 * kvh), (causal ? 2.0 : 4.0) * B * (double)T * T * heads * hd,
        launch_attn_prefill(a, s));
    return OPUS_OK;
}

extern "C" int opus_debug_attn_prefill(opus_ctx *c, const void *Q, const void *K, const void *V, void *O, int64_t q_st, int64_t k_st,
                                       int64_t v_st, int64_t o_st, int64_t q_sb, int64_t k_sb, int64_t v_sb, int64_t o_sb,
                                       const int32_t *kstart, const int32_t *kend, const int32_t *cu, int32_t B, int32_t T,
                                       int32_t heads, int32_t group, int32_t hd, int32_t causal, int32_t q_trim, float scale,
                                       int32_t *qt_used, void *stream) {
    if (qt_used) *qt_used = 0;
    if (!c || !Q || !K || !V || !O || !qt_used) return fail(OPUS_EBADARG, "debug_attn_prefill: null pointer");
    if (B < 1 || T < 1 || heads < 1 || group < 1 || heads % group || hd < 1) return fail(OPUS_ESHAPE, "debug_attn_prefill: shape");
// ... 194 lines not shown
```

opus-pllm_amd/csrc/common.h:

```cpp
#pragma once
#include <hip/hip_runtime.h>
#include <hip/hip_ext.h>
#include <stdint.h>

namespace opus {

#ifdef OPUS_BF16
typedef __bf16 half_t;
typedef __bf16 h8 __attribute__((ext_vector_type(8)));
typedef __bf16 h4 __attribute__((ext_vector_type(4)));
typedef __bf16 h2 __attribute__((ext_vector_type(2)));
#else
typedef _Float16 half_t;
typedef _Float16 h8 __attribute__((ext_vector_type(8)));
typedef _Float16 h4 __attribute__((ext_vector_type(4)));
typedef _Float16 h2 __attribute__((ext_vector_type(2)));
#endif
typedef float f4 __attribute__((ext_vector_type(4)));
__device__ __forceinline__ f4 mfma16(h8 a, h8 b, f4 c) {
#ifdef OPUS_BF16
    return __builtin_amdgcn_mfma_f32_16x16x32_bf16(a, b, c, 0, 0, 0);
#else
    return __builtin_amdgcn_mfma_f32_16x16x32_f16(a, b, c, 0, 0, 0);
#endif
// ... 92 lines not shown
    int epi;
    float *ws;
    int64_t ws_bytes;
    half_t *xh_out;
    float *ssq_out;
    int *fused_done;
    const float *row_ssq;
    int row_nblk;
    int64_t ssq_cap = 0;
    int *nblk_out = nullptr;
    int slab_only = 0;
    int *ks_out = nullptr;
    int force_wide = 0;
    const float *rope_cs = nullptr;
    const int32_t *rope_pos = nullptr;
    int rope_T = 0, rope_cols = 0, rope_qcols = 0;
    float rope_qscale = 1.0f;
    int *rope_done = nullptr;
    int a_tiled = 0, xh_tiled = 0, c_tiled = 0;
    int *combine_cnt = nullptr;
    float *ln_part = nullptr;
    int *ln_done = nullptr;
    const float *ln_stat = nullptr;
    const float *ln_colsum = nullptr;
    int pp_gm = 8;
    int stagger = 0;
    int no_rot = 0;
    long long *trace = nullptr;
    int *pp_plan = nullptr;
    int *plan = nullptr;
    const uint8_t *q8 = nullptr;
    const int8_t *e8 = nullptr;
    int *ran_w8 = nullptr;
};
constexpr int PP_PLAN_WORDS = 5;
enum PpTail { PP_TAIL_NONE = 0, PP_TAIL_PAIR = 1, PP_TAIL_REDUCE = 2 };
constexpr int GEMM_PLAN_WORDS = 8;
enum GemmCombine { GC_NONE = 0, GC_REDUCE = 1, GC_REDUCE4 = 2, GC_IN_LAUNCH = 3, GC_PP_PAIR = 4, GC_PP_REDUCE = 5, GC_SLABS = 6 };
inline void gemm_plan_set(const GemmParams &p, int klass, int mt, int tn, int ns, int alds, int P, int ks, int combine) {
    if (!p.plan) return;
    const int v[GEMM_PLAN_WORDS] = {klass, mt, tn, ns, alds, P, ks, combine};
    for (int i = 0; i < GEMM_PLAN_WORDS; ++i) p.plan[i] = v[i];
}

struct AttnParams {
    const half_t *Q, *K, *V;
    int64_t q_sb, q_st, k_sb, k_st, v_sb, v_st;
    half_t *O;
    int64_t o_sb, o_st;
    const int32_t *kstart;
    const int32_t *kend;
    int B, T, heads, group, head_dim, causal;
    float scale;
    const int32_t *cu = nullptr;
    int q_trim = 0;
};

hipError_t launch_gemm(const GemmParams &p, hipStream_t s, int *klass);
hipError_t launch_splitk_reduce(const GemmParams &p, int ks, hipStream_t s);
bool gemm_stream_ok(const GemmParams &p);
bool gemm_stream_would(int M, int N, int K, int slab_only, int a_tiled, int row_scale, int64_t ws_bytes);
hipError_t launch_gemm_stream(const GemmParams &p, hipStream_t s);
struct Knobs {
    int no_stream = 0;
    int no_ln_fusion = 0;
    int debug_a_tiled = 0;
// ... 132 lines not shown
hipError_t launch_gather_rows2(const float *x, int64_t n_x, const float *y, int64_t n_y, const int32_t *rows, int R, int H, float *out,
                               hipStream_t s);
hipError_t launch_xent(const half_t *logits, int64_t ld, int R, int V, const int32_t *targets, float *logprob, float *lse,
                       hipStream_t s);
hipError_t launch_tree_edges(const half_t *logits, int64_t ld, const float *lse, int row0, const int32_t *erow, const int32_t *etok,
                             const int32_t *eslot, int n_edges, float *node_lp, const int32_t *srow, const int32_t *sset,
                             const int32_t *sslot, int n_stops, const int32_t *ids, const int32_t *soff, float *stop_lp, hipStream_t s);
hipError_t launch_tree_path_sums(const float *node_lp, const int32_t *trie, const int32_t *par, const int32_t *depth,
                                 const int32_t *mnode, int P, int M, int ld_nodes, float *member_lp, hipStream_t s);
hipError_t launch_relu_h(half_t *x, int64_t n, hipStream_t s);
hipError_t launch_fill_synth(void *dst, int dtype, int64_t rows, int64_t cols, uint64_t seed, float std,
                             float mean, int64_t rb, int64_t rs, int64_t ro, int tiled, uint64_t fold_seed,
                             float fold_std, float fold_mean, hipStream_t s);
hipError_t launch_argmax_partial(const float *logits, int B, int V, float *pval, int32_t *pidx, hipStream_t s);
hipError_t launch_tile_weight(const half_t *src, half_t *dst, int64_t N, int64_t K, hipStream_t s);
hipError_t launch_lora_merge(half_t *W, const half_t *A, const half_t *B, float scale, int64_t out_f,
                             int64_t in_f, int r, hipStream_t s);
hipError_t launch_splice_plan(const int64_t *ids, const uint8_t *mask, int B, int Tt, int n_tok, int max_len,
                              int V, int32_t *plan, hipStream_t s);
hipError_t launch_splice_fill(const int64_t *ids, const uint8_t *mask, int B, int Tt, const half_t *prot,
                              int n_tok, int H, int V, const half_t *emb, const int32_t *plan, int Tout,
                              int left_pad, half_t *out, uint8_t *mask_out, int32_t *pos_out, hipStream_t s);
hipError_t launch_sample_select(const float *logits, int B, int V, float temperature, float top_p, int top_k, const uint64_t *seed,
                                const int32_t *step, float *pmax, int32_t *pidx, float *cand_p, int32_t *cand_i,
                                int32_t *cand_n, float *zpart, float *spart, int32_t *chosen, float *thr_out, float *psum,
                                float *thr_keep, hipStream_t s);
constexpr int APART = 64;
__device__ __forceinline__ uint64_t splitmix64(uint64_t x) {
    x += 0x9E3779B97F4A7C15ull;
    x = (x ^ (x >> 30)) * 0xBF58476D1CE4E5B9ull;
    x = (x ^ (x >> 27)) * 0x94D049BB133111EBull;
    return x ^ (x >> 31);
}
hipError_t launch_argmax_step(const float *pval, const int32_t *pidx, const int32_t *chosen, int B, const int32_t *eos, int n_eos, int pad_id,
                              int32_t *finished, int32_t *out_ids, int max_new, const int32_t *step,
                              int32_t *next_tok, int32_t *n_unfinished, const int32_t *stop, int n_stop, hipStream_t s);
hipError_t launch_step_advance(int32_t *step, hipStream_t s);
struct GenOutDesc {
    float *token_lp;
    float *scores;
    float *logits;
    float *unused;
};
hipError_t launch_argmax_lse_partial(const float *logits, int B, int V, float *pval, int32_t *pidx, float *psum, hipStream_t s);
hipError_t launch_argmax_lse_step(const float *pval, const int32_t *pidx, const float *psum, const int32_t *chosen, int B,
                                  const int32_t *eos, int n_eos, int pad_id, int32_t *finished, int32_t *out_ids, int max_new,
                                  const int32_t *step, int32_t *next_tok, int32_t *n_unfinished, const int32_t *stop, int n_stop,
                                  const float *logits, int V, const GenOutDesc *out, hipStream_t s);
hipError_t launch_argmax_lse_final(const float *pval, const int32_t *pidx, const float *psum, int B, int32_t *idx, float *lse,
                                   hipStream_t s);
hipError_t launch_argmax_rawlp_step(const float *pval, const int32_t *pidx, const float *lse, const float *raw_hist,
                                    const int32_t *chosen, int B, const int32_t *eos, int n_eos, int pad_id, int32_t *finished,
                                    int32_t *out_ids, int max_new, const int32_t *step, int32_t *next_tok, int32_t *n_unfinished,
                                    const int32_t *stop, int n_stop, const float *logits, int V, const GenOutDesc *out,
                                    hipStream_t s);
hipError_t launch_gen_scores(const float *logits, int B, int V, const GenOutDesc *out, const int32_t *step, int max_new,
                             float temperature, float top_p, const float *pmax, const float *thr, hipStream_t s);
constexpr int LP_MAX_BAD = 256, LP_MAX_BAD_LEN = 8, LP_MAX_BAD_IDS = 1024, LP_MAX_HIST = 2048;
struct LogitsProcDesc {
    float penalty;
    int32_t ngram;
    int32_t min_new;
    int32_t n_bad;
    int32_t bad_off[LP_MAX_BAD + 1];
    int32_t bad_ids[LP_MAX_BAD_IDS];
};
hipError_t launch_logits_proc(float *logits, int B, int V, const int32_t *hist, int64_t ld, const int32_t *step, int max_hist,
                              const int32_t *eos, int n_eos, const LogitsProcDesc *desc, float *raw_hist, hipStream_t s);
constexpr int TC_MAX_VOCAB = 1 << 18, TC_MAX_END = 64;
struct TokenConstraintDesc {
    const int32_t *edge_off;
    const int32_t *edge_tok;
    const int32_t *edge_next;
    const uint8_t *completing;
    const int32_t *end_ids;
    const int32_t *start;
    int32_t *state;
    int32_t n_states, n_end, n_start, state_stride;
    int32_t start_div, unused;
};
hipError_t launch_token_constraint(float *logits, int B, int V, const int32_t *hist, int64_t ld, const int32_t *step, int max_hist,
                                   const TokenConstraintDesc *desc, hipStream_t s);
hipError_t launch_guidance_lse_partial(const float *logits, int B, int V, float *pval, float *psum, hipStream_t s);
hipError_t launch_guidance_lse_final(const float *pval, const float *psum, int B, float *rmax, float *rlog, float *rlse, hipStream_t s);
hipError_t launch_guidance_combine(float *cond, const float *uncond, int n, int V, const float *max_c, const float *log_c,
                                   const float *max_u, const float *log_u, const float *g, float *keep, hipStream_t s);
hipError_t launch_guidance_pair_next(int32_t *next, int P, hipStream_t s);
hipError_t launch_beam_topk(const float *logits, const float *run, int B, int K, int V, int M, float *lse, float *out_s,
                            int32_t *out_i, hipStream_t s);
hipError_t launch_beam_sample(const float *logits, const float *run, int B, int K, int V, int M, float temperature, const float *pmax,
                              const float *thr, int min_keep, float *kth_s, int32_t *kth_i, uint64_t seed, int step, float *lse,
                              float *out_s, int32_t *out_i, hipStream_t s);
hipError_t launch_kv_gather_rows(half_t *cache, half_t *tmp, const int32_t *idx, int R, int64_t row_halfs, int nsub, int64_t sub_halfs,
                                 const int32_t *step, int T0, int hd, int back, hipStream_t s);
hipError_t launch_upload_i32(const int32_t *h, int n, int32_t *dst, hipStream_t s);
hipError_t launch_mask_to_kstart(const uint8_t *mask, int B, int T, int32_t *kstart, hipStream_t s);

struct LookupAcceptParams {
    const int32_t *y;
    const int32_t *x;
    int ld_x;
    const int32_t *draft_len;
    int R, n;
    int pre;
    int32_t *ids;
    int stride;
    int32_t *fin;
    const int32_t *eos, *stop;
    int n_eos, n_stop, pad;
    int32_t *step;
    int32_t *next;
    int32_t *n_unf;
    int32_t *words;
    int32_t *max_len;
};
// ... 36 lines not shown
```

opus-pllm_amd/csrc/constraint.hip:

```cpp
#include "common.h"

namespace opus {

constexpr int TC_THREADS = 1024;

__global__ __launch_bounds__(TC_THREADS) void token_constraint_kernel(float *__restrict__ logits, int V, int chunk,
                                                                      const int32_t *__restrict__ hist, int64_t ld,
                                                                      const int32_t *__restrict__ step, int max_hist,
                                                                      const TokenConstraintDesc *__restrict__ dp) {
    extern __shared__ uint32_t s_map[];
    __shared__ int32_t s_state;
    const int b = blockIdx.x, tid = threadIdx.x;
    const TokenConstraintDesc d = *dp;
    if (tid == 0) {
        int t = *step;
        t = t < 0 ? 0 : (t > max_hist ? max_hist : t);
        int s;
        if (t == 0) {
            s = d.start[d.n_start > 1 ? b / d.start_div : 0];
        } else {
            int cur = d.state[((t - 1) & 1) * d.state_stride + b];
            if ((unsigned)cur >= (unsigned)d.n_states) cur = 0;
            const int tok = hist[(int64_t)b * ld + t - 1];
            int lo = d.edge_off[cur], hi = d.edge_off[cur + 1];
            while (lo < hi) {
                const int mid = (lo + hi) >> 1;
                if (d.edge_tok[mid] < tok) lo = mid + 1; else hi = mid;
            }
            s = (lo < d.edge_off[cur + 1] && d.edge_tok[lo] == tok) ? d.edge_next[lo] : 0;
        }
        if ((unsigned)s >= (unsigned)d.n_states) s = 0;
        if (blockIdx.y == 0) d.state[(t & 1) * d.state_stride + b] = s;
        s_state = s;
    }
    if (!logits) return;
    const int lo = blockIdx.y * chunk, hi = min(V, lo + chunk);
    if (lo >= hi) return;
    const int wbase = lo >> 5, nw = ((hi - 1) >> 5) - wbase + 1;
    for (int w = tid; w <= nw; w += TC_THREADS) s_map[w] = 0u;
    __syncthreads();
    const int s = s_state;
    const int e0 = d.edge_off[s], e1 = d.edge_off[s + 1];
    for (int e = e0 + tid; e < e1; e += TC_THREADS) {
        const int id = d.edge_tok[e];
        if (id >= lo && id < hi) atomicOr(&s_map[(id >> 5) - wbase], 1u << (id & 31));
    }
    if (d.completing[s])
        for (int k = tid; k < d.n_end; k += TC_THREADS) {
            const int id = d.end_ids[k];
            if (id >= lo && id < hi) atomicOr(&s_map[(id >> 5) - wbase], 1u << (id & 31));
        }
    __syncthreads();

    float *row = logits + (int64_t)b * V;
    const float ninf = -INFINITY;
    const int r0 = (int)(((16u - (unsigned)(reinterpret_cast<uintptr_t>(row) & 15u)) & 15u) >> 2);
    const int i0 = min(hi, lo + ((r0 - lo) & 3));
    const int n4 = (hi - i0) >> 2;
    if (tid < i0 - lo) {
        const int i = lo + tid;
        if (!((s_map[(i >> 5) - wbase] >> (i & 31)) & 1u)) row[i] = ninf;
    }
    for (int q = tid; q < n4; q += TC_THREADS) {
        const int i = i0 + 4 * q;
        const int w = (i >> 5) - wbase, sh = i & 31;
        uint32_t bits = s_map[w] >> sh;
        if (sh > 28) bits |= s_map[w + 1] << (32 - sh);
        bits &= 0xfu;
        if (bits == 0u) {
            *reinterpret_cast<float4 *>(row + i) = make_float4(ninf, ninf, ninf, ninf);
        } else if (bits != 0xfu) {
#pragma unroll
            for (int k = 0; k < 4; ++k)
                if (!((bits >> k) & 1u)) row[i + k] = ninf;
        }
    }
    const int t0 = i0 + 4 * n4;
    if (tid < hi - t0) {
        const int i = t0 + tid;
        if (!((s_map[(i >> 5) - wbase] >> (i & 31)) & 1u)) row[i] = ninf;
    }
}

hipError_t launch_token_constraint(float *logits, int B, int V, const int32_t *hist, int64_t ld, const int32_t *step, int max_hist,
                                   const TokenConstraintDesc *desc, hipStream_t s) {
    if (V < 1 || V > TC_MAX_VOCAB || B < 1) return hipErrorInvalidValue;
    int P = logits ? 256 / B : 1;
    P = P < 1 ? 1 : (P > 8 ? 8 : P);
    const int chunk = ((V + P - 1) / P + 31) & ~31;
    const size_t lds = logits ? (size_t)(chunk / 32 + 1) * sizeof(uint32_t) : 0;
    hipLaunchKernelGGL(token_constraint_kernel, dim3(B, P), dim3(TC_THREADS), lds, s, logits, V, chunk, hist, ld, step, max_hist, desc);
    return hipGetLastError();
}

}
```

opus-pllm_amd/csrc/elementwise.hip:

```cpp
#include "common.h"

namespace opus {

__global__ __launch_bounds__(256) void esm_embed_kernel(const int32_t *__restrict__ tok, const half_t *__restrict__ emb,
                                                        int T, int D, float *__restrict__ x, const int32_t *__restrict__ cu,
                                                        int32_t *__restrict__ pos) {
    __shared__ int s_cnt[2];
    const int b = blockIdx.y;
    int64_t r0 = (int64_t)b * T;
    if (cu) {
        r0 = cu[b];
        T = cu[b + 1] - cu[b];
        if ((int)blockIdx.x * 16 >= T) return;
    }
    const int32_t *row = tok + r0;
    if (threadIdx.x < 2) s_cnt[threadIdx.x] = 0;
    __syncthreads();
    int nm = 0, nv = 0;
    for (int t = threadIdx.x; t < T; t += 256) {
        const int v = row[t];
        nm += (v == 32);
        nv += (v != 1);
    }
    atomicAdd(&s_cnt[0], nm);
// ... 520 lines not shown
    }
    s_v[threadIdx.x] = bv;
    s_i[threadIdx.x] = bi;
    s_s[threadIdx.x] = bs;
    __syncthreads();
    for (int o = 128; o > 0; o >>= 1) {
        if (threadIdx.x < o) {
            const float v = s_v[threadIdx.x + o], m = s_v[threadIdx.x];
            const int i = s_i[threadIdx.x + o];
            const float M = fmaxf(m, v);
            s_s[threadIdx.x] = M == -INFINITY ? 0.f : s_s[threadIdx.x] * __expf(m - M) + s_s[threadIdx.x + o] * __expf(v - M);
            if (v > m || (v == m && i < s_i[threadIdx.x])) {
                s_v[threadIdx.x] = v;
                s_i[threadIdx.x] = i;
            }
        }
        __syncthreads();
    }
    if (threadIdx.x == 0) {
        pval[b * APART + part] = s_v[0];
        pidx[b * APART + part] = s_i[0];
        psum[b * APART + part] = s_s[0];
    }
}

__device__ __forceinline__ float parts_lse(float mp, float sp, float M) {
    float e = mp > -INFINITY ? sp * __expf(mp - M) : 0.f;
#pragma unroll
    for (int o = 32; o > 0; o >>= 1) e += __shfl_xor(e, o, 64);
    return M + logf(e);
}

template <int LP>
__device__ __forceinline__ void argmax_step_body(const float *__restrict__ pval, const int32_t *__restrict__ pidx,
                                                 const int32_t *__restrict__ chosen, const int32_t *__restrict__ eos, int n_eos,
                                                 int pad_id, int32_t *__restrict__ finished, int32_t *__restrict__ out_ids,
                                                 int max_new, const int32_t *__restrict__ step, int32_t *__restrict__ next_tok,
                                                 int32_t *__restrict__ n_unf, const int32_t *__restrict__ stop, int n_stop,
                                                 const float *__restrict__ logits, int V, const float *__restrict__ psum,
                                                 const GenOutDesc *__restrict__ out, const float *__restrict__ lse_in = nullptr,
                                                 const float *__restrict__ raw_hist = nullptr) {
    const int b = blockIdx.x, lane = threadIdx.x;
    float bv = pval[b * APART + lane];
    int bi = pidx[b * APART + lane];
    const float mp = bv, sp = LP == 1 ? psum[b * APART + lane] : 0.f;
#pragma unroll
    for (int o = 32; o > 0; o >>= 1) {
        const float v = __shfl_xor(bv, o, 64);
        const int i = __shfl_xor(bi, o, 64);
        if (v > bv || (v == bv && i < bi)) { bv = v; bi = i; }
    }
    float lse = LP == 1 ? parts_lse(mp, sp, bv) : 0.f;
    if (chosen) bi = chosen[b];
    float raw_tok = 0.f;
    if (LP == 2) {
        const int st = *step, n = st < max_new ? st : max_new;
        const int tok = finished[b] ? pad_id : (bi == 0x7fffffff ? 0 : bi);
        int first = 0x7fffffff;
        if (raw_hist)
            for (int i = lane; i < n; i += 64)
                if (out_ids[(int64_t)b * max_new + i] == tok) { first = i; break; }
#pragma unroll
        for (int o = 32; o > 0; o >>= 1) first = min(first, __shfl_xor(first, o, 64));
        lse = lse_in[b];
        raw_tok = first != 0x7fffffff ? raw_hist[(int64_t)b * max_new + first]
                                      : ((unsigned)tok < (unsigned)V ? logits[(int64_t)b * V + tok] : NAN);
    }
    if (lane == 0) {
        const int st = *step;
        int fin = finished[b];
        int tok = fin ? pad_id : (bi == 0x7fffffff ? 0 : bi);
        if (st < max_new) out_ids[(int64_t)b * max_new + st] = tok;
        if (LP == 1 && st < max_new)
            out->token_lp[(int64_t)b * max_new + st] =
                fin ? 0.f : ((unsigned)tok < (unsigned)V ? logits[(int64_t)b * V + tok] - lse : NAN);
        if (LP == 2 && st < max_new) out->token_lp[(int64_t)b * max_new + st] = fin ? 0.f : raw_tok - lse;
        if (!fin)
            for (int e = 0; e < n_eos; ++e) fin |= (tok == eos[e]);
        if (!fin && n_stop > 0 && st + 1 >= n_stop && st < max_new) {
            bool hit = true;
            for (int k = 0; k < n_stop; ++k) hit = hit && out_ids[(int64_t)b * max_new + st - n_stop + 1 + k] == stop[k];
            fin |= hit ? 1 : 0;
        }
        finished[b] = fin;
        next_tok[b] = tok;
        if (!fin && st < max_new) atomicAdd(&n_unf[st], 1);
    }
}
__global__ __launch_bounds__(64) void argmax_step_kernel(const float *__restrict__ pval, const int32_t *__restrict__ pidx,
                                                         const int32_t *__restrict__ chosen,
                                                         const int32_t *__restrict__ eos, int n_eos, int pad_id,
                                                         int32_t *__restrict__ finished, int32_t *__restrict__ out_ids,
                                                         int max_new, const int32_t *__restrict__ step,
                                                         int32_t *__restrict__ next_tok, int32_t *__restrict__ n_unf,
                                                         const int32_t *__restrict__ stop, int n_stop) {
    argmax_step_body<0>(pval, pidx, chosen, eos, n_eos, pad_id, finished, out_ids, max_new, step, next_tok, n_unf, stop, n_stop,
                            nullptr, 0, nullptr, nullptr);
}
__global__ __launch_bounds__(64) void argmax_lse_step_kernel(const float *__restrict__ pval, const int32_t *__restrict__ pidx,
                                                             const int32_t *__restrict__ chosen,
                                                             const int32_t *__restrict__ eos, int n_eos, int pad_id,
                                                             int32_t *__restrict__ finished, int32_t *__restrict__ out_ids,
                                                             int max_new, const int32_t *__restrict__ step,
                                                             int32_t *__restrict__ next_tok, int32_t *__restrict__ n_unf,
                                                             const int32_t *__restrict__ stop, int n_stop,
                                                             const float *__restrict__ logits, int V, const float *__restrict__ psum,
                                                             const GenOutDesc *__restrict__ out) {
    argmax_step_body<1>(pval, pidx, chosen, eos, n_eos, pad_id, finished, out_ids, max_new, step, next_tok, n_unf, stop, n_stop,
                           logits, V, psum, out);
}
__global__ __launch_bounds__(64) void argmax_rawlp_step_kernel(const float *__restrict__ pval, const int32_t *__restrict__ pidx,
                                                               const int32_t *__restrict__ chosen,
                                                               const int32_t *__restrict__ eos, int n_eos, int pad_id,
                                                               int32_t *__restrict__ finished, int32_t *__restrict__ out_ids,
                                                               int max_new, const int32_t *__restrict__ step,
                                                               int32_t *__restrict__ next_tok, int32_t *__restrict__ n_unf,
                                                               const int32_t *__restrict__ stop, int n_stop,
                                                               const float *__restrict__ logits, int V, const GenOutDesc *__restrict__ out,
                                                               const float *__restrict__ lse, const float *__restrict__ raw_hist) {
    argmax_step_body<2>(pval, pidx, chosen, eos, n_eos, pad_id, finished, out_ids, max_new, step, next_tok, n_unf, stop, n_stop,
                        logits, V, nullptr, out, lse, raw_hist);
}
hipError_t launch_argmax_rawlp_step(const float *pval, const int32_t *pidx, const float *lse, const float *raw_hist,
                                    const int32_t *chosen, int B, const int32_t *eos, int n_eos, int pad_id, int32_t *finished,
                                    int32_t *out_ids, int max_new, const int32_t *step, int32_t *next_tok, int32_t *n_unfinished,
                                    const int32_t *stop, int n_stop, const float *logits, int V, const GenOutDesc *out,
                                    hipStream_t s) {
    hipLaunchKernelGGL(argmax_rawlp_step_kernel, dim3(B), dim3(64), 0, s, pval, pidx, chosen, eos, n_eos, pad_id, finished, out_ids,
                       max_new, step, next_tok, n_unfinished, stop, n_stop, logits, V, out, lse, raw_hist);
    return hipGetLastError();
}
hipError_t launch_argmax_step(const float *pval, const int32_t *pidx, const int32_t *chosen, int B, const int32_t *eos,
                              int n_eos, int pad_id, int32_t *finished, int32_t *out_ids, int max_new, const int32_t *step,
                              int32_t *next_tok, int32_t *n_unfinished, const int32_t *stop, int n_stop, hipStream_t s) {
    hipLaunchKernelGGL(argmax_step_kernel, dim3(B), dim3(64), 0, s, pval, pidx, chosen, eos, n_eos, pad_id, finished, out_ids,
                       max_new, step, next_tok, n_unfinished, stop, n_stop);
    return hipGetLastError();
}
hipError_t launch_argmax_lse_partial(const float *logits, int B, int V, float *pval, int32_t *pidx, float *psum, hipStream_t s) {
    hipLaunchKernelGGL(argmax_lse_partial_kernel, dim3(APART, B), dim3(256), 0, s, logits, V, pval, pidx, psum);
    return hipGetLastError();
}
hipError_t launch_argmax_lse_step(const float *pval, const int32_t *pidx, const float *psum, const int32_t *chosen, int B,
                                  const int32_t *eos, int n_eos, int pad_id, int32_t *finished, int32_t *out_ids, int max_new,
                                  const int32_t *step, int32_t *next_tok, int32_t *n_unfinished, const int32_t *stop, int n_stop,
                                  const float *logits, int V, const GenOutDesc *out, hipStream_t s) {
    hipLaunchKernelGGL(argmax_lse_step_kernel, dim3(B), dim3(64), 0, s, pval, pidx, chosen, eos, n_eos, pad_id, finished, out_ids,
                       max_new, step, next_tok, n_unfinished, stop, n_stop, logits, V, psum, out);
    return hipGetLastError();
}

__global__ __launch_bounds__(64) void argmax_lse_final_kernel(const float *__restrict__ pval, const int32_t *__restrict__ pidx,
                                                              const float *__restrict__ psum, int32_t *__restrict__ idx,
                                                              float *__restrict__ lse) {
    const int b = blockIdx.x, lane = threadIdx.x;
    float bv = pval[b * APART + lane];
    int bi = pidx[b * APART + lane];
    const float mp = bv, sp = psum[b * APART + lane];
#pragma unroll
    for (int o = 32; o > 0; o >>= 1) {
        const float v = __shfl_xor(bv, o, 64);
        const int i = __shfl_xor(bi, o, 64);
        if (v > bv || (v == bv && i < bi)) { bv = v; bi = i; }
    }
    const float l = parts_lse(mp, sp, bv);
    if (lane == 0) {
        idx[b] = bi;
        lse[b] = l;
    }
}
hipError_t launch_argmax_lse_final(const float *pval, const int32_t *pidx, const float *psum, int B, int32_t *idx, float *lse,
                                   hipStream_t s) {
    hipLaunchKernelGGL(argmax_lse_final_kernel, dim3(B), dim3(64), 0, s, pval, pidx, psum, idx, lse);
    return hipGetLastError();
}

constexpr int GS_CHUNK = 4096;
__global__ __launch_bounds__(256) void gen_scores_kernel(const float *__restrict__ logits, int V, const GenOutDesc *__restrict__ out,
                                                         const int32_t *__restrict__ step, int max_new, float inv_temp, float top_p,
                                                         const float *__restrict__ pmax, const float *__restrict__ thr) {
// ... 389 lines not shown
```

opus-pllm_amd/csrc/gemm.hip:

```cpp
#include "common.h"
#include <cstdlib>
#include <map>
#include <type_traits>
#include <mutex>
#include <utility>

namespace opus {

thread_local LaunchEvents *tl_launch_ev = nullptr;
static Knobs knobs_from_env() {
    Knobs k;
    for (int i = 0; i < 8; ++i) {
        char name[32];
        snprintf(name, sizeof(name), "OPUS_KNOB_MISC%d", i);
        if (const char *v = getenv(name)) k.misc[i] = atoi(v);
    }
    return k;
}
Knobs g_knobs = knobs_from_env();

hipError_t ensure_dyn_lds(const void *fn, size_t bytes) {
    static std::mutex mu;
    static std::map<std::pair<int, const void *>, size_t> done;
    int dev = 0;
// ... 2065 lines not shown
            }
        }
        return;
    }
    if (p.row_ssq) {
#pragma unroll
        for (int i = 0; i < MT; ++i) {
            const float rs = rstd_s[16 * i + li];
#pragma unroll
            for (int r = 0; r < 4; ++r) acc[i][r] *= rs;
        }
    }
    if (EPI == EPI_SILU_GU16) {
        __syncthreads();
        float *xch = reinterpret_cast<float *>(smem);
        if (wave & 1) {
#pragma unroll
            for (int i = 0; i < MT; ++i)
#pragma unroll
                for (int r = 0; r < 4; ++r) xch[(((wave >> 1) * MT + i) * 4 + r) * 64 + lane] = acc[i][r];
        }
        __syncthreads();
        if ((wave & 1) == 0 && panel_ok) {
#pragma unroll
            for (int i = 0; i < MT; ++i) {
                const int m = 16 * i + li;
                if (m >= p.M) continue;
                f4 up;
#pragma unroll
                for (int r = 0; r < 4; ++r) up[r] = xch[(((wave >> 1) * MT + i) * 4 + r) * 64 + lane];
                store4<EPI>(p, m, panel * 16 + 4 * g, acc[i], up);
            }
        }
    } else if (panel_ok) {
#pragma unroll
        for (int i = 0; i < MT; ++i) {
            const int m = 16 * i + li;
            if (m < p.M) store4<EPI>(p, m, panel * 16 + 4 * g, acc[i], acc[i]);
        }
    }
}

template <int MT, int EPI, bool W8 = false>
static hipError_t launch_wide(const GemmParams &p, hipStream_t s) {
    if constexpr (!W8) {
        if (p.q8 && p.e8) return launch_wide<MT, EPI, true>(p, s);
    }
    const int blocks = cdiv((p.N + 15) >> 4, 8), chunks = p.K / 64;
    int ks = 1;
    if (p.ws && blocks < 200) {
        ks = 256 / blocks;
        ks = ks > 8 ? 8 : ks;
        if (ks > chunks / 8) ks = chunks / 8;
        while (ks > 1 && (int64_t)ks * p.M * p.N * 4 > p.ws_bytes) --ks;
        if (ks < 1) ks = 1;
    }
    if (p.ks_out) *p.ks_out = ks;
    const int lds = 2 * (MT <= 4 ? 8 : 4) * 16 * MT * 128 + 16 * MT * (int)sizeof(float);
    hipError_t ea = ensure_dyn_lds(reinterpret_cast<const void *>(&gemm_wide_kernel<MT, EPI, W8>), lds);
    if (ea != hipSuccess) return ea;
    gemm_plan_set(p, KC_WIDE, MT, 0, 0, 0, 0, ks, ks == 1 ? GC_NONE : GC_SLABS);
    if (W8 && p.ran_w8) *p.ran_w8 = 1;
    if (ks > 1 && p.row_ssq) {
        GemmParams q = p;
        q.row_ssq = nullptr;
        OPUS_LAUNCH(KC_WIDE, (gemm_wide_kernel<MT, EPI, W8>), dim3(blocks, ks), dim3(512), lds, s, q, ks);
    } else {
        OPUS_LAUNCH(KC_WIDE, (gemm_wide_kernel<MT, EPI, W8>), dim3(blocks, ks), dim3(512), lds, s, p, ks);
    }
    hipError_t e = hipGetLastError();
    if (e != hipSuccess || ks == 1 || p.slab_only) return e;
    return launch_reduce<EPI>(p, ks, s);
}


template <int MT, int EPI, bool NORM, bool W8 = false>
static hipError_t launch_mid_t(const GemmParams &p, hipStream_t s) {
    if constexpr (!W8 && MT <= 4) {
        if (p.q8 && p.e8) return launch_mid_t<MT, EPI, NORM, true>(p, s);
    }
    const int blocks = cdiv((p.N + 15) >> 4, 4), chunks = p.K / 64;
    int ks = 1;
    if (p.ws && blocks < 384) {
        ks = cdiv(512, blocks);
        ks = ks > 8 ? 8 : ks;
        if (ks > chunks / 4) ks = chunks / 4;
        while (ks > 1 && ((int64_t)ks * p.M * p.N + (int64_t)ks * p.M) * 4 > p.ws_bytes) --ks;
        if (ks < 1) ks = 1;
    }
    constexpr int CH = MT <= 2 ? 4 : 1;
    const size_t lds = 2 * CH * 16 * MT * 128 + 16 * MT * sizeof(float) + 2 * MT * 4 * 64 * sizeof(float);
    if (lds > 48 * 1024) {
        hipError_t ea = ensure_dyn_lds(reinterpret_cast<const void *>(&gemm_mid_kernel<MT, EPI, NORM, W8>), lds);
        if (ea != hipSuccess) return ea;
    }
    if (p.row_ssq && ks == 1) return hipErrorInvalidValue;
    gemm_plan_set(p, KC_MID, MT, 0, 0, 0, 0, ks, GC_NONE);
    if (W8 && p.ran_w8) *p.ran_w8 = 1;
// ... 93 lines not shown

bool gemm_goes_wide(int M, int N) {
    static const bool no_mid = getenv("OPUS_NO_MID_GEMM") != nullptr, mid_v1 = getenv("OPUS_MID_V1") != nullptr;
    if (mid_v1 || N < 16384 || M <= SKINNY_MAX_M || M > 96) return false;
    return M > MID_MAX_M || !no_mid;
}

static hipError_t launch_gemm_(const GemmParams &p, hipStream_t s, int *klass);
hipError_t launch_gemm(const GemmParams &p, hipStream_t s, int *klass) {
    static const bool no_rot = getenv("OPUS_NO_KROT") != nullptr;
    if (!no_rot) return launch_gemm_(p, s, klass);
    GemmParams q = p;
    q.no_rot = 1;
    return launch_gemm_(q, s, klass);
}
static bool pp_min_tiles_ok(int M, int N) {
    static const bool no_big = getenv("OPUS_NO_BIG_GEMM") != nullptr, no_pp = getenv("OPUS_NO_PP") != nullptr;
    static const int min_tiles = getenv("OPUS_PP_MIN_TILES") ? atoi(getenv("OPUS_PP_MIN_TILES")) : 128;
    return !no_big && !no_pp && (int64_t)cdiv(M, 256) * cdiv(N, 256) >= min_tiles;
}
bool gemm_goes_pp(int M, int N) { return M > 96 && pp_min_tiles_ok(M, N); }

static hipError_t launch_gemm_(const GemmParams &p, hipStream_t s, int *klass) {
    if (p.ln_stat && !gemm_goes_pp(p.M, p.N)) return hipErrorInvalidValue;
    if (p.M <= 0 || p.N <= 0 || p.K <= 0 || (p.K & 63) || (p.lda & 7)) return hipErrorInvalidValue;
    if (p.epi == EPI_SILU_GU16 && (p.N & 31)) return hipErrorInvalidValue;
    const bool skinny = p.M <= SKINNY_MAX_M;
    static const bool no_mid = getenv("OPUS_NO_MID_GEMM") != nullptr;
    const bool mid = !skinny && p.M <= MID_MAX_M && !no_mid;
    static const bool mid_v1 = getenv("OPUS_MID_V1") != nullptr;
    if (klass) *klass = skinny ? KC_SKINNY : KC_TILE;
    if (p.Af && !skinny && !mid) return hipErrorInvalidValue;
    if (p.Af && p.epi == EPI_GELU) return hipErrorInvalidValue;
    const bool to_stream = mid && !p.Af && p.N < 16384 && gemm_stream_ok(p);
    const bool to_wide = !to_stream && mid && !p.Af && !mid_v1 && (p.N >= 16384 || p.force_wide || narrow_wide());
    if (p.a_tiled && !to_stream) return hipErrorInvalidValue;
    if (p.c_tiled && (p.out_f32 || !(to_stream || to_wide) || ((p.epi == EPI_SILU_GU16 ? p.N / 2 : p.N) & 63))) return hipErrorInvalidValue;
    if (p.row_ssq && skinny) return hipErrorInvalidValue;
    if (skinny) {
        if (p.Af) {
            switch (p.epi) {
                case EPI_NONE: return launch_skinny_e<EPI_NONE, true>(p, s);
                case EPI_SILU_GU16: return launch_skinny_e<EPI_SILU_GU16, true>(p, s);
            }
            return hipErrorInvalidValue;
        }
        switch (p.epi) {
            case EPI_NONE: return launch_skinny_e<EPI_NONE, false>(p, s);
            case EPI_GELU: return launch_skinny_e<EPI_GELU, false>(p, s);
            case EPI_SILU_GU16: return launch_skinny_e<EPI_SILU_GU16, false>(p, s);
        }
    } else if (mid && !p.Af && !mid_v1 && p.N < 16384 && gemm_stream_ok(p)) {
        return launch_gemm_stream(p, s);
    } else if (mid && !p.Af && !mid_v1 && (p.N >= 16384 || p.force_wide || narrow_wide())) {
        const bool m2 = p.M <= 32;
        switch (p.epi) {
            case EPI_NONE: return m2 ? launch_wide<2, EPI_NONE>(p, s) : launch_wide<4, EPI_NONE>(p, s);
            case EPI_GELU: return m2 ? launch_wide<2, EPI_GELU>(p, s) : launch_wide<4, EPI_GELU>(p, s);
            case EPI_SILU_GU16: return m2 ? launch_wide<2, EPI_SILU_GU16>(p, s) : launch_wide<4, EPI_SILU_GU16>(p, s);
        }
    } else if (mid && !p.Af && !mid_v1 && p.M > 32) {
        switch (p.epi) {
            case EPI_NONE: return launch_ring<2, 2, 8, EPI_NONE>(p, s, true);
            case EPI_GELU: return launch_ring<2, 2, 8, EPI_GELU>(p, s, true);
            case EPI_SILU_GU16: return launch_ring<2, 2, 8, EPI_SILU_GU16>(p, s, true);
        }
    } else if (mid) {
        if (p.Af) {
            switch (p.epi) {
                case EPI_NONE: return launch_mid_e<EPI_NONE, true>(p, s);
                case EPI_SILU_GU16: return launch_mid_e<EPI_SILU_GU16, true>(p, s);
            }
            return hipErrorInvalidValue;
        }
        switch (p.epi) {
            case EPI_NONE: return launch_mid_e<EPI_NONE, false>(p, s);
            case EPI_GELU: return launch_mid_e<EPI_GELU, false>(p, s);
            case EPI_SILU_GU16: return launch_mid_e<EPI_SILU_GU16, false>(p, s);
        }
    } else if (!p.Af && p.M <= 96 && p.N >= 16384 && !mid_v1) {
        switch (p.epi) {
            case EPI_NONE: return launch_wide<6, EPI_NONE>(p, s);
            case EPI_GELU: return launch_wide<6, EPI_GELU>(p, s);
            case EPI_SILU_GU16: return launch_wide<6, EPI_SILU_GU16>(p, s);
        }
    } else {
        switch (p.epi) {
// ... 10 lines not shown
```

opus-pllm_amd/eval_ddp.py:

```python
#!/usr/bin/env python3
from __future__ import annotations

import argparse
import json
import os
import sys
import time

import torch

sys.path.insert(0, os.path.dirname(os.path.dirname(os.path.abspath(__file__))))
import opus_pllm_amd as opa
from opus_pllm_amd import dist as odist
from opus_pllm_amd.builder import load_pretrained_model, return_cstp_path
from opus_pllm_amd.prompt import (add_constraint_args, add_logits_processor_args, add_lookup_args, after_process_output,
                                  build_prompt, logits_processor_kwargs, lookup_kwargs, max_new_tokens_for, token_constraint)


def annotate(model, tokenizer, items, input_path, batch_size, max_new, temperature=0.0, top_p=0.7, num_beams=1,
             use_input_embed=False, device=None, logits_out=None, stop_sequence=None, inflight=1, logprobs_out=None,
             processors=None, num_return_sequences=1, share_prompt_head=False, guidance_scale=None):
    dev = device or model.device
    nret = int(num_return_sequences)
    if nret < 1:
# ... 7 lines not shown
    if use_input_embed and items:
        prot_all = model.project_dataset(torch.tensor([q["input_embed"] for q in items], dtype=torch.float32, device=dev))
    starts = list(range(0, len(items), batch_size))
    head_len, head = 0, None
    if share_prompt_head and items:
        head_len = shared_head_length([opa.tokenizer_seq_token(build_prompt(q["instruction"], input_path), tokenizer,
                                                               opa.DEFAULT_SEQ_TOKEN_INDEX) for q in items])
        if head_len:
            first = opa.tokenizer_seq_token(build_prompt(items[0]["instruction"], input_path), tokenizer, opa.DEFAULT_SEQ_TOKEN_INDEX)
            with torch.inference_mode():
                head = model.cache_prefix(torch.tensor([list(first[:head_len])], dtype=torch.long, device=dev), detach=True)
    outs = [None] * len(starts)
    last = [None] * len(starts)
    lps = [None] * len(starts)
    seeds = [int(torch.randint(0, 2 ** 62, (1,)).item()) for _ in starts] if temperature > 0 else [None] * len(starts)

    def one(m, j):
        i = starts[j]
        batch = items[i:i + batch_size]
        prompts = [build_prompt(q["instruction"], input_path) for q in batch]
        ids = [opa.tokenizer_seq_token(p, tokenizer, opa.DEFAULT_SEQ_TOKEN_INDEX, return_tensors="pt").to(dev)[head_len:] for p in prompts]
        ids = opa.left_pad_sequence(ids, padding_value=tokenizer.pad_token_id, batch_first=True)
        mask = ids != tokenizer.pad_token_id
        extra = {} if prot_all is None else {"protein_tokens": prot_all[i:i + len(batch)]}
        extra.update(processors or {})
        if head is not None:
            extra.update(prefix=head, prefix_rows=[0] * len(batch))
        if nret > 1:
            extra["num_return_sequences"] = nret
        if guided:
            extra["guidance_scale"] = float(guidance_scale)
        if logprobs_out is not None:
            extra.update(return_dict_in_generate=True, output_token_logprobs=True)
        with torch.inference_mode():
            out = m.generate(ids, [q["input"] for q in batch], attention_mask=mask, pad_token_id=tokenizer.eos_token_id,
                             do_sample=temperature > 0, temperature=temperature, top_p=top_p,
                             num_beams=num_beams, max_new_tokens=max_new, use_cache=True, stop_sequence=stop_sequence,
                             seed=seeds[j], **extra)
        if logprobs_out is not None:
            lp = torch.zeros((out.sequences.shape[0], max_new), dtype=torch.float32, device=dev)
            lp[:, : out.token_logprobs.shape[1]] = out.token_logprobs
            lps[j] = (lp, out.n_tokens)
            out = out.sequences
        if logits_out is not None:
            last[j] = m.last_logits(len(batch) * nret)
        full = torch.full((out.shape[0], max_new), tokenizer.eos_token_id, dtype=torch.long, device=dev)
        full[:, : out.shape[1]] = out
        outs[j] = full

    n_ctx = max(1, min(int(inflight), len(starts)))
    if n_ctx == 1:
        for j in range(len(starts)):
            one(model, j)
    else:
        import threading
        ctxs = [model] + [model.new_context() for _ in range(n_ctx - 1)]
        errs = []

        def worker(k):
            try:
                torch.cuda.set_device(dev)
                with torch.cuda.stream(torch.cuda.Stream(dev)):
                    for j in range(k, len(starts), n_ctx):
                        one(ctxs[k], j)
                    torch.cuda.current_stream(dev).synchronize()
            except BaseException as e:
# ... 304 lines not shown
```

opus-pllm_amd/model.py:

```python
from __future__ import annotations

import ctypes as C
import types
from typing import List, Optional, Sequence, Union

import numpy as np
import torch

from . import _cabi
from .alphabet import batch_convert, batch_convert_packed, encode_array, pack_token_arrays
from .config import OpusConfig
from .constants import DEFAULT_SEQ_TOKEN_INDEX, IGNORE_INDEX
from .weights import DeviceWeights


class _ProteinEncoderHandle:

    def __init__(self, owner: "OpusLlamaForCausalLM"):
        self._owner = owner

    def get_protein_seq_embeddings(self, data: Sequence[str]) -> torch.Tensor:
        return self._owner._encode(list(data))

    def get_amino_acid_embeddings(self, data, return_contacts: bool = False):
# ... 1332 lines not shown
    def last_hidden(self, B: int, T: int) -> torch.Tensor:
        s = self._enter()
        with torch.cuda.stream(self._stream):
            h = torch.empty((B, T, self.cfg.enc_dim), dtype=torch.float32, device=self.device)
            _cabi.check(self._lib.opus_esm2_last_hidden(self._ctx, h.data_ptr(), B, T, s))
        self._leave()
        return h

    def timing(self, on: bool):
        _cabi.check(self._lib.opus_timing_enable(self._ctx, 1 if on else 0))
        _cabi.check(self._lib.opus_timing_reset(self._ctx))

    def timing_get(self, klass: str = "*", phase: str = "*"):
        ms, n, by, fl = C.c_double(0), C.c_int64(0), C.c_double(0), C.c_double(0)
        _cabi.check(self._lib.opus_timing_get(self._ctx, klass.encode(), phase.encode(), C.byref(ms), C.byref(n), C.byref(by),
                                              C.byref(fl)))
        return ms.value, n.value, by.value, fl.value

    def timing_names(self):
        buf = C.create_string_buffer(512)
        _cabi.check(self._lib.opus_timing_names(buf, 512))
        classes, phases = buf.value.decode().split(";")
        return classes.split(","), phases.split(",")

    def drop_decode_graphs(self) -> None:
        _cabi.check(self._lib.opus_debug_knob(self._ctx, b"misc0", 0))

    def stat(self, name: str) -> int:
        v = int(self._lib.opus_stat(self._ctx, name.encode()))
        if v < 0:
            raise KeyError(name)
        return v

    def last_logits(self, B: int) -> torch.Tensor:
        s = self._enter()
        with torch.cuda.stream(self._stream):
            out = torch.empty((B, self.cfg.dec_vocab), dtype=torch.float32, device=self.device)
            _cabi.check(self._lib.opus_last_logits(self._ctx, out.data_ptr(), B, s))
        self._leave()
        return out


def _splice_labels(input_ids, attention_mask, labels, n_tok, T_out, inference_mode):
    ids = input_ids.cpu()
    lab = labels.cpu()
    m = torch.ones_like(ids, dtype=torch.bool) if attention_mask is None else attention_mask.cpu().bool()
    out = torch.full((ids.shape[0], T_out), IGNORE_INDEX, dtype=lab.dtype)
    for b in range(ids.shape[0]):
        row: List[int] = []
        for t in range(ids.shape[1]):
            if not m[b, t]:
                continue
            if int(ids[b, t]) == DEFAULT_SEQ_TOKEN_INDEX:
                row.extend([IGNORE_INDEX] * n_tok)
            else:
                row.append(int(lab[b, t]))
        row = row[:T_out]
        if row:
            if inference_mode:
                out[b, T_out - len(row):] = torch.tensor(row, dtype=lab.dtype)
            else:
                out[b, : len(row)] = torch.tensor(row, dtype=lab.dtype)
    return out


def _check_forward_mask(m: np.ndarray, pos: Optional[np.ndarray]) -> None:
# ... 445 lines not shown
```

Measured before the change: 259.8 proteins/s.

## Fuse greedy argmax into LM-head GEMM epilogue and skip logits store

For greedy decoding without logits processors, the LM-head wide GEMM now computes per-block row argmax in its epilogue and writes partial max values and indices instead of storing the full fp32 logits. The separate argmax_partial pass is skipped, and argmax_step reduces over the per-128-column groups. This removes the write and re-read of a B×vocab fp32 logits tensor each step. In exchange the K-split of the wide kernel is disabled (whole-K), which can lower parallelism on the large-vocab GEMM. A keep_last_logits flag is added so callers that need the raw logits can opt out.

```diff
diff --git a/include/opus_pllm.h b/include/opus_pllm.h
--- a/include/opus_pllm.h
+++ b/include/opus_pllm.h
@@ -198,6 +198,8 @@
 
 int opus_debug_gemm(opus_ctx *ctx, const void *d_A, const void *d_W, const float *d_bias, const float *d_residual,
                     void *d_C, int32_t M, int32_t N, int32_t K, int32_t epi, int32_t out_f32, void *stream);
+int opus_debug_gemm_pick(opus_ctx *ctx, const void *d_A, const void *d_W, const float *d_bias, float *d_C, int32_t M, int32_t N,
+                         int32_t K, float *d_val, int32_t *d_idx, int32_t store, void *stream);
 int opus_debug_gemm_norm(opus_ctx *ctx, const float *d_A, const void *d_W, void *d_C, int32_t M, int32_t N, int32_t K,
                          int32_t epi, int32_t out_f32, float eps, void *stream);
 int opus_debug_gemm_slabs(opus_ctx *ctx, const void *d_A, const void *d_W, float *d_slabs, int32_t M, int32_t N, int32_t K,
@@ -256,6 +258,7 @@
                             int32_t poison, void *stream);
 
 int opus_last_logits(opus_ctx *ctx, float *d_out, int32_t B, void *stream);
+int opus_keep_last_logits(opus_ctx *ctx, int32_t on);
 
 int64_t opus_stat(opus_ctx *ctx, const char *name);
 
diff --git a/opus-pllm_amd/_cabi.py b/opus-pllm_amd/_cabi.py
--- a/opus-pllm_amd/_cabi.py
+++ b/opus-pllm_amd/_cabi.py
@@ -121,6 +121,8 @@
                                   C.POINTER(C.c_double), C.POINTER(C.c_double)]),
     "opus_timing_names": (C.c_int, [C.c_char_p, C.c_int32]),
     "opus_last_logits": (C.c_int, [_P, _P, C.c_int32, _P]),
+    "opus_keep_last_logits": (C.c_int, [_P, C.c_int32]),
+    "opus_debug_gemm_pick": (C.c_int, [_P, _P, _P, _P, _P, C.c_int32, C.c_int32, C.c_int32, _P, _P, C.c_int32, _P]),
     "opus_check_error": (C.c_int, [_P, _P]),
     "opus_beam_topk": (C.c_int, [_P, _P, C.c_int32, C.c_int32, C.c_int32, _P, _P, _P]),
     "opus_kv_reorder": (C.c_int, [_P, _P, C.c_int32, _P]),
diff --git a/opus-pllm_amd/csrc/api.cpp b/opus-pllm_amd/csrc/api.cpp
--- a/opus-pllm_amd/csrc/api.cpp
+++ b/opus-pllm_amd/csrc/api.cpp
@@ -71,11 +71,12 @@
     bool lproc = false;
     bool cons = false;
     int budget = -1;
+    bool fused_head = false;
 };
 static bool same_step(const StepPlan &a, const StepPlan &b) {
     return a.rows == b.rows && a.guided == b.guided && a.stride == b.stride && a.ids == b.ids && a.n_eos == b.n_eos && a.pad == b.pad &&
            a.temp == b.temp && a.top_p == b.top_p && a.top_k == b.top_k && a.n_stop == b.n_stop && a.outs == b.outs &&
-           a.lproc == b.lproc && a.cons == b.cons && a.budget == b.budget;
+           a.lproc == b.lproc && a.cons == b.cons && a.budget == b.budget && a.fused_head == b.fused_head;
 }
 
 struct opus_ctx {
@@ -102,6 +103,8 @@
     uint64_t *d_seed;
     int32_t *d_chosen;
     int samp_top_k = 0;
+    bool keep_logits = false;
+    bool logits_stale = false;
     float *d_bthr = nullptr, *d_blse = nullptr;
     int64_t gemm_ws_bytes = 0;
     half_t *d_xn, *d_qkv, *d_ctx, *d_act, *d_xln, *kc, *vc;
@@ -126,6 +129,9 @@
     int64_t graph_replays = 0;
     int64_t decode_steps = 0;
     char *gen_mem = nullptr;
+    char *head_mem = nullptr;
+    float *d_hval = nullptr;
+    int32_t *d_hidx = nullptr;
     GenOutDesc *d_gen = nullptr;
     GenOutDesc h_gen{};
     float *d_gpsum = nullptr, *d_gthr = nullptr;
@@ -402,6 +408,7 @@
     if (c->proj_big) (void)hipFree(c->proj_big);
     if (c->kv_tmp) (void)hipFree(c->kv_tmp);
     if (c->gen_mem) (void)hipFree(c->gen_mem);
+    if (c->head_mem) (void)hipFree(c->head_mem);
     if (c->lproc_mem) (void)hipFree(c->lproc_mem);
     if (c->cons_tab) (void)hipFree(c->cons_tab);
     if (c->cons_mem) (void)hipFree(c->cons_mem);
@@ -587,6 +594,10 @@
     int *pp_plan = nullptr;
     const uint8_t *q8 = nullptr;
     const int8_t *e8 = nullptr;
+    float *pick_val = nullptr;
+    int32_t *pick_idx = nullptr;
+    int pick_ld = 0, pick_only = 0;
+    int whole_k = 0;
     GemmAsk &copy16(half_t *dst, bool tiled = false) { xh = dst; xh_tiled = dst && tiled; return *this; }
     GemmAsk &scale_rows(float eps, int nblk) { rs_on = true; rs_eps = eps; rs_nblk = nblk; return *this; }
     GemmAsk &rope(const float *cs, const int32_t *pos, int T, int D, float qscale) {
@@ -600,9 +611,11 @@
     GemmAsk &tiled_c(int on) { c_tiled = on; return *this; }
     GemmAsk &report_pp(int *plan) { pp_plan = plan; return *this; }
     GemmAsk &w8(const uint8_t *q, const int8_t *e) { if (q && e) { q8 = q; e8 = e; } return *this; }
+    GemmAsk &pick(float *val, int32_t *idx, int ld, bool only) { if (val && idx) { pick_val = val; pick_idx = idx; pick_ld = ld; pick_only = only; } return *this; }
+    GemmAsk &wide_whole_k() { whole_k = 1; return *this; }
 };
 struct GemmGot {
-    int xh_done = 0, rope_done = 0, ln_done = 0, ks = 1, ssq_nblk = 0;
+    int xh_done = 0, rope_done = 0, ln_done = 0, ks = 1, ssq_nblk = 0, picked = 0;
 };
 
 static int gemm_any(opus_ctx *c, hipStream_t s, const half_t *A, const float *Af, float eps, int64_t lda, const half_t *W,
@@ -630,8 +643,11 @@
     c->gemm_w8 = 0;
     p.q8 = ask.q8; p.e8 = ask.e8; p.ran_w8 = &c->gemm_w8;
     p.a_tiled = ask.a_tiled; p.xh_tiled = ask.xh_tiled; p.c_tiled = ask.c_tiled;
+    p.amax_val = ask.pick_val; p.amax_idx = ask.pick_idx; p.amax_ld = ask.pick_ld; p.amax_nostore = ask.pick_only;
+    p.amax_done = &got->picked; p.wide_whole_k = ask.whole_k;
     const int nout = epi == EPI_SILU_GU16 ? N / 2 : N;
-    const double bytes = 2.0 * N * K + (Af ? 4.0 : 2.0) * M * K + (double)M * nout * (out_f32 ? 4 : 2) +
+    const double bytes = 2.0 * N * K + (Af ? 4.0 : 2.0) * M * K +
+                         (ask.pick_val && ask.pick_only ? 8.0 * M * ask.pick_ld : (double)M * nout * (out_f32 ? 4 : 2)) +
                          (residual ? 4.0 * M * nout : 0.0);
     int klass = M <= SKINNY_MAX_M ? KC_SKINNY : KC_TILE;
     hipError_t e;
@@ -640,6 +656,8 @@
         e = launch_gemm(p, s, &klass);
     }
     if (e != hipSuccess) return fail(OPUS_EHIP, "gemm M=%d N=%d K=%d failed: %s", M, N, K, hipGetErrorString(e));
+    if (ask.pick_val && ask.pick_only && !got->picked)
+        return fail(OPUS_EHIP, "gemm M=%d N=%d K=%d: the launch took a kernel without the fused pick its caller planned on", M, N, K);
     c->w8_gemms += c->gemm_w8;
     return OPUS_OK;
 }
@@ -1141,10 +1159,16 @@
     return OPUS_OK;
 }
 
-static int lm_head(opus_ctx *c, hipStream_t s, ResidShadow &sh, int B, float *out = nullptr) {
-    const opus_config &g = c->cfg;
+static int head_groups(const opus_ctx *c) { return cdiv(c->cfg.dec_vocab, 128); }
+static bool head_picks(const opus_ctx *c, const StepPlan &p) {
+    return p.temp == 0.f && !p.lproc && !p.cons && !p.guided && p.outs == 0 && p.budget < 0 && !c->keep_logits && !g_knobs.misc[2] &&
+           c->cfg.dec_arch == 0 && p.rows <= MID_MAX_M && gemm_goes_wide(p.rows, c->cfg.dec_vocab);
+}
+static int lm_head(opus_ctx *c, hipStream_t s, ResidShadow &sh, int B, float *out = nullptr, bool pick = false) {
+    const opus_config &g = c->cfg;
+    c->logits_stale = pick;
     return gemm_norm(c, s, sh, c->d_xl, g.dec_rms_eps, c->d_xln, c->lm_head, B, g.dec_vocab, g.dec_dim, EPI_NONE, out ? out : c->d_logits,
-                     g.dec_vocab, 1);
+                     g.dec_vocab, 1, nullptr, GemmAsk().pick(pick ? c->d_hval : nullptr, c->d_hidx, head_groups(c), true));
 }
 
 static int fanout_rows(opus_ctx *c, hipStream_t s, int B, int nret) {
@@ -1252,6 +1276,7 @@
 
 static int lm_head_opt(opus_ctx *c, hipStream_t s, int B, float *out = nullptr) {
     const opus_config &g = c->cfg;
+    c->logits_stale = false;
     KL(KC_NORM, 6.0 * B * g.dec_dim, launch_layernorm(c->d_xl, c->dec_lnfw, c->dec_lnfb, g.dec_rms_eps, B, g.dec_dim, c->d_xln, nullptr, s));
     return gemm(c, s, c->d_xln, g.dec_dim, c->lm_head, B, g.dec_vocab, g.dec_dim, nullptr, EPI_NONE, nullptr, out ? out : c->d_logits,
                 g.dec_vocab, 1);
@@ -1281,7 +1306,7 @@
 }
 
 static int prefill(opus_ctx *c, hipStream_t s, const half_t *embeds, const uint8_t *mask, int B, int T, bool all_rows = false,
-                   const ContRows *cont = nullptr, int nret = 1) {
+                   const ContRows *cont = nullptr, int nret = 1, bool pick = false) {
     c->phase = cont && !cont->app_lens ? PH_SCORE : PH_PREFILL;
     if (cont && cont->w8) c->phase = PH_DECODE;
     if (cont) {
@@ -1355,10 +1380,10 @@
         if (have_stat) OPC(finalize());
     }
     if (all_rows) return OPUS_OK;
-    return finish_prefill(c, s, B, T, nret, last_rows_done, [&](float *out) { return lm_head(c, s, sh, B, out); });
-}
-
-static int decode_step(opus_ctx *c, hipStream_t s, const int32_t *d_tok) {
+    return finish_prefill(c, s, B, T, nret, last_rows_done, [&](float *out) { return lm_head(c, s, sh, B, out, pick && nret == 1); });
+}
+
+static int decode_step(opus_ctx *c, hipStream_t s, const int32_t *d_tok, bool pick = false) {
     c->phase = PH_DECODE;
     const opus_config &g = c->cfg;
     const int B = c->cur_B, T = c->cur_T;
@@ -1397,7 +1422,7 @@
         OPC(gemm(c, s, c->d_act, F, L.wd, B, H, F, nullptr, EPI_NONE, c->d_xl, c->d_xl, H, 1, GemmAsk().copy16(copy_xl, next_tiled).tiled_a(act_tiled).w8(L.q8_d, L.e8_d), &got));
         sh.produced(c->d_xl, got, next_tiled);
     }
-    OPC(lm_head(c, s, sh, B));
+    OPC(lm_head(c, s, sh, B, nullptr, pick));
     KL(KC_OTHER, 8.0, launch_step_advance(c->d_step, s));
     return OPUS_OK;
 }
@@ -2157,6 +2182,15 @@
     return OPUS_OK;
 }
 
+static int ensure_head_mem(opus_ctx *c) {
+    if (c->head_mem) return OPUS_OK;
+    const size_t one = align_up((size_t)c->cfg.max_batch * head_groups(c) * sizeof(float));
+    HIPC(hipMalloc((void **)&c->head_mem, 2 * one));
+    c->d_hval = reinterpret_cast<float *>(c->head_mem);
+    c->d_hidx = reinterpret_cast<int32_t *>(c->head_mem + one);
+    return OPUS_OK;
+}
+
 static int ensure_lproc_mem(opus_ctx *c) {
     if (c->lproc_mem) return OPUS_OK;
     const size_t B = c->cfg.max_batch, N = c->cfg.max_new_tokens;
@@ -2226,6 +2260,7 @@
     const bool proc = p.lproc || p.cons || guid;
     const bool lp = p.outs & GEN_LOGPROBS, sc = p.outs & (GEN_SCORES | GEN_LOGITS);
     const size_t BV = (size_t)HB * g.dec_vocab;
+    const bool cons_picks = p.cons && !p.lproc && !guid && p.temp == 0.f && p.outs == 0 && !g_knobs.misc[2];
     if (proc) {
         if (p.outs & GEN_LOGITS)
             KL(KC_OTHER, 8.0 * BV, launch_gen_scores(c->d_logits, HB, g.dec_vocab, c->d_gen_raw, c->d_step, max_new, 0.f, 1.f,
@@ -2246,7 +2281,8 @@
                                   lp && !guid ? c->d_rawh : nullptr, s));
         if (p.cons)
             KL(KC_CONSTRAINT, 4.0 * BV,
-               launch_token_constraint(c->d_logits, HB, g.dec_vocab, d_out, max_new, c->d_step, max_new, c->d_cons, s));
+               launch_token_constraint(c->d_logits, HB, g.dec_vocab, d_out, max_new, c->d_step, max_new, c->d_cons, s,
+                                       cons_picks ? c->d_pval : nullptr, c->d_pidx));
     }
     if (p.temp > 0.f) {
         KL(KC_OTHER, 4.0 * 4 * HB * g.dec_vocab,
@@ -2257,25 +2293,28 @@
     } else if (lp && !proc) {
         KL(KC_OTHER, 4.0 * HB * g.dec_vocab,
            launch_argmax_lse_partial(c->d_logits, HB, g.dec_vocab, c->d_pval, c->d_pidx, c->d_gpsum, s));
-    } else {
+    } else if (!p.fused_head && !cons_picks) {
         KL(KC_OTHER, 4.0 * HB * g.dec_vocab, launch_argmax_partial(c->d_logits, HB, g.dec_vocab, c->d_pval, c->d_pidx, s));
     }
+    const int nparts = p.fused_head ? head_groups(c) : (cons_picks ? token_constraint_slices(HB) : APART);
+    const float *pval = p.fused_head ? c->d_hval : c->d_pval;
+    const int32_t *pidx = p.fused_head ? c->d_hidx : c->d_pidx;
     if (proc ? (p.outs & GEN_SCORES) != 0 : sc)
         KL(KC_OTHER, 4.0 * HB * g.dec_vocab * (1 + ((p.outs & GEN_SCORES) ? 1 : 0) + ((p.outs & GEN_LOGITS) && !proc ? 1 : 0)),
            launch_gen_scores(c->d_logits, HB, g.dec_vocab, proc ? c->d_gen_proc : c->d_gen, c->d_step, max_new, p.temp,
                              p.top_p, c->d_pval, p.temp > 0.f ? c->d_gthr : nullptr, s));
     if (lp && proc)
         KL(KC_OTHER, 512.0 * HB + 8.0 * HB * max_new,
-           launch_argmax_rawlp_step(c->d_pval, c->d_pidx, guid ? c->d_glse : c->d_rlse, p.lproc && !guid ? c->d_rawh : nullptr, chosen, HB, c->d_eos, n_eos, pad_id, c->d_fin, d_out,
+           launch_argmax_rawlp_step(c->d_pval, c->d_pidx, APART, guid ? c->d_glse : c->d_rlse, p.lproc && !guid ? c->d_rawh : nullptr, chosen, HB, c->d_eos, n_eos, pad_id, c->d_fin, d_out,
                                     max_new, c->d_step, c->d_next, c->d_nunf, c->d_stop, p.n_stop, guid ? c->guid_keep : c->d_logits,
                                     g.dec_vocab, c->d_gen_proc, s));
     else if (lp)
         KL(KC_OTHER, 512.0 * HB + 8.0 * HB,
-           launch_argmax_lse_step(c->d_pval, c->d_pidx, c->d_gpsum, chosen, HB, c->d_eos, n_eos, pad_id, c->d_fin, d_out, max_new,
+           launch_argmax_lse_step(c->d_pval, c->d_pidx, APART, c->d_gpsum, chosen, HB, c->d_eos, n_eos, pad_id, c->d_fin, d_out, max_new,
                                   c->d_step, c->d_next, c->d_nunf, c->d_stop, p.n_stop, c->d_logits, g.dec_vocab, c->d_gen, s));
     else
-        KL(KC_OTHER, 512.0 * HB,
-           launch_argmax_step(c->d_pval, c->d_pidx, chosen, HB, c->d_eos, n_eos, pad_id, c->d_fin, d_out, max_new, c->d_step,
+        KL(KC_OTHER, 8.0 * nparts * HB,
+           launch_argmax_step(pval, pidx, nparts, chosen, HB, c->d_eos, n_eos, pad_id, c->d_fin, d_out, max_new, c->d_step,
                               c->d_next, c->d_nunf, c->d_stop, p.n_stop, s));
     if (guid) KL(KC_GUIDANCE, 8.0 * HB, launch_guidance_pair_next(c->d_next, HB, s));
     return OPUS_OK;
@@ -2283,7 +2322,7 @@
 
 static int greedy_body(opus_ctx *c, hipStream_t s, const StepPlan &p) {
     OPC(select_next(c, s, p));
-    return decode_step(c, s, c->d_next);
+    return decode_step(c, s, c->d_next, p.fused_head);
 }
 
 static int capture_step(opus_ctx *c, hipStream_t s, int (*body)(opus_ctx *, hipStream_t, const StepPlan &), const StepPlan &p,
@@ -2340,6 +2379,8 @@
     plan.temp = temperature; plan.top_p = top_p; plan.top_k = c->samp_top_k; plan.n_stop = c->n_stop;
     plan.lproc = c->lproc_on; plan.cons = c->cons_on;
     if (outs) plan.outs = (outs->token_lp ? GEN_LOGPROBS : 0) | (outs->scores ? GEN_SCORES : 0) | (outs->logits ? GEN_LOGITS : 0);
+    plan.fused_head = !behind && nret == 1 && head_picks(c, plan);
+    if (plan.fused_head) OPC(ensure_head_mem(c));
     if (plan.outs) {
         OPC(ensure_gen_mem(c));
         c->h_gen = *outs;
@@ -2364,7 +2405,7 @@
         }
     }
     if (behind) OPC(prefill_behind(c, s, *behind, (const half_t *)d_embeds, B, T));
-    else OPC(prefill(c, s, (const half_t *)d_embeds, d_mask, B, T, false, nullptr, nret));
+    else OPC(prefill(c, s, (const half_t *)d_embeds, d_mask, B, T, false, nullptr, nret, plan.fused_head));
 
     const bool use_graph = s != nullptr && !c->timing && !getenv("OPUS_NO_GRAPH");
     opus_ctx::GraphEntry *ge = nullptr;
@@ -2930,9 +2971,11 @@
     c->phase = PH_DECODE;
     if (g.dec_arch == 1) {
         KL(KC_NORM, 6.0 * M * H, launch_layernorm(c->d_x, c->dec_lnfw, c->dec_lnfb, g.dec_rms_eps, M, H, c->d_xn, nullptr, s));
+        c->logits_stale = false;
         OPC(gemm(c, s, c->d_xn, H, c->lm_head, M, V, H, nullptr, EPI_NONE, nullptr, c->d_logits, V, 1));
     } else {
         ResidShadow none;
+        c->logits_stale = false;
         OPC(gemm_norm(c, s, none, c->d_x, g.dec_rms_eps, c->d_xn, c->lm_head, M, V, H, EPI_NONE, c->d_logits, V, 1));
     }
     ++c->lookup_passes;
@@ -3146,6 +3189,20 @@
                 out_f32, GemmAsk().tiled_a(g_knobs.debug_a_tiled));
 }
 
+extern "C" int opus_debug_gemm_pick(opus_ctx *c, const void *A, const void *W, const float *bias, float *Cp, int32_t M, int32_t N,
+                                    int32_t K, float *d_val, int32_t *d_idx, int32_t store, void *stream) {
+    if (!c || !A || !W || !Cp || !d_val || !d_idx) return fail(OPUS_EBADARG, "debug_gemm_pick: null pointer");
+    if (M <= SKINNY_MAX_M || M > MID_MAX_M || N < 1 || K < 64 || K % 64)
+        return fail(OPUS_ESHAPE, "debug_gemm_pick: %d < M <= %d, K a positive multiple of 64", SKINNY_MAX_M, MID_MAX_M);
+    HIPC(hipSetDevice(c->device));
+    GemmAsk ask = GemmAsk().wide_whole_k();
+    if (!g_knobs.misc[2]) ask.pick(d_val, d_idx, cdiv(N, 128), !store);
+    GemmGot got;
+    OPC(gemm(c, (hipStream_t)stream, (const half_t *)A, K, (const half_t *)W, M, N, K, bias, EPI_NONE, nullptr, Cp, N, 1, ask, &got));
+    if (!g_knobs.misc[2] && !got.picked) return fail(OPUS_EHIP, "debug_gemm_pick: the launch did not pick");
+    return OPUS_OK;
+}
+
 extern "C" int opus_debug_gemm_norm(opus_ctx *c, const float *A, const void *W, void *Cp, int32_t M, int32_t N, int32_t K,
                                     int32_t epi, int32_t out_f32, float eps, void *stream) {
     if (!c || !A || !W || !Cp) return fail(OPUS_EBADARG, "debug_gemm_norm: null pointer");
@@ -3358,10 +3415,18 @@
     return OPUS_OK;
 }
 
+extern "C" int opus_keep_last_logits(opus_ctx *c, int32_t on) {
+    if (!c) return fail(OPUS_EBADARG, "ctx is null");
+    c->keep_logits = on != 0;
+    return OPUS_OK;
+}
+
 extern "C" int opus_last_logits(opus_ctx *c, float *d_out, int32_t B, void *stream) {
     if (!c || !d_out) return fail(OPUS_EBADARG, "last_logits: null pointer");
     if (!c->prefilled) return fail(OPUS_ESTATE, "last_logits before prefill");
     if (B < 1 || B > c->cur_B) return fail(OPUS_ESHAPE, "last_logits: B=%d but the last prefill had %d rows", B, c->cur_B);
+    if (c->logits_stale)
+        return fail(OPUS_ESTATE, "last_logits: the last greedy step picked in its lm_head and stored no logits (opus_keep_last_logits)");
     HIPC(hipSetDevice(c->device));
     HIPC(hipMemcpyAsync(d_out, c->d_logits, (size_t)B * c->cfg.dec_vocab * sizeof(float), hipMemcpyDeviceToDevice, (hipStream_t)stream));
     return OPUS_OK;
diff --git a/opus-pllm_amd/csrc/common.h b/opus-pllm_amd/csrc/common.h
--- a/opus-pllm_amd/csrc/common.h
+++ b/opus-pllm_amd/csrc/common.h
@@ -148,6 +148,11 @@
     const uint8_t *q8 = nullptr;
     const int8_t *e8 = nullptr;
     int *ran_w8 = nullptr;
+    float *amax_val = nullptr;
+    int32_t *amax_idx = nullptr;
+    int amax_ld = 0, amax_nostore = 0;
+    int *amax_done = nullptr;
+    int wide_whole_k = 0;
 };
 constexpr int PP_PLAN_WORDS = 5;
 enum PpTail { PP_TAIL_NONE = 0, PP_TAIL_PAIR = 1, PP_TAIL_REDUCE = 2 };
@@ -346,7 +351,7 @@
     x = (x ^ (x >> 27)) * 0x94D049BB133111EBull;
     return x ^ (x >> 31);
 }
-hipError_t launch_argmax_step(const float *pval, const int32_t *pidx, const int32_t *chosen, int B, const int32_t *eos, int n_eos, int pad_id,
+hipError_t launch_argmax_step(const float *pval, const int32_t *pidx, int nparts, const int32_t *chosen, int B, const int32_t *eos, int n_eos, int pad_id,
                               int32_t *finished, int32_t *out_ids, int max_new, const int32_t *step,
                               int32_t *next_tok, int32_t *n_unfinished, const int32_t *stop, int n_stop, hipStream_t s);
 hipError_t launch_step_advance(int32_t *step, hipStream_t s);
@@ -357,13 +362,13 @@
     float *unused;
 };
 hipError_t launch_argmax_lse_partial(const float *logits, int B, int V, float *pval, int32_t *pidx, float *psum, hipStream_t s);
-hipError_t launch_argmax_lse_step(const float *pval, const int32_t *pidx, const float *psum, const int32_t *chosen, int B,
+hipError_t launch_argmax_lse_step(const float *pval, const int32_t *pidx, int nparts, const float *psum, const int32_t *chosen, int B,
                                   const int32_t *eos, int n_eos, int pad_id, int32_t *finished, int32_t *out_ids, int max_new,
                                   const int32_t *step, int32_t *next_tok, int32_t *n_unfinished, const int32_t *stop, int n_stop,
                                   const float *logits, int V, const GenOutDesc *out, hipStream_t s);
 hipError_t launch_argmax_lse_final(const float *pval, const int32_t *pidx, const float *psum, int B, int32_t *idx, float *lse,
                                    hipStream_t s);
-hipError_t launch_argmax_rawlp_step(const float *pval, const int32_t *pidx, const float *lse, const float *raw_hist,
+hipError_t launch_argmax_rawlp_step(const float *pval, const int32_t *pidx, int nparts, const float *lse, const float *raw_hist,
                                     const int32_t *chosen, int B, const int32_t *eos, int n_eos, int pad_id, int32_t *finished,
                                     int32_t *out_ids, int max_new, const int32_t *step, int32_t *next_tok, int32_t *n_unfinished,
                                     const int32_t *stop, int n_stop, const float *logits, int V, const GenOutDesc *out,
@@ -394,7 +399,8 @@
     int32_t start_div, unused;
 };
 hipError_t launch_token_constraint(float *logits, int B, int V, const int32_t *hist, int64_t ld, const int32_t *step, int max_hist,
-                                   const TokenConstraintDesc *desc, hipStream_t s);
+                                   const TokenConstraintDesc *desc, hipStream_t s, float *pval = nullptr, int32_t *pidx = nullptr);
+int token_constraint_slices(int B);
 hipError_t launch_guidance_lse_partial(const float *logits, int B, int V, float *pval, float *psum, hipStream_t s);
 hipError_t launch_guidance_lse_final(const float *pval, const float *psum, int B, float *rmax, float *rlog, float *rlse, hipStream_t s);
 hipError_t launch_guidance_combine(float *cond, const float *uncond, int n, int V, const float *max_c, const float *log_c,
diff --git a/opus-pllm_amd/csrc/constraint.hip b/opus-pllm_amd/csrc/constraint.hip
--- a/opus-pllm_amd/csrc/constraint.hip
+++ b/opus-pllm_amd/csrc/constraint.hip
@@ -7,9 +7,12 @@
 __global__ __launch_bounds__(TC_THREADS) void token_constraint_kernel(float *__restrict__ logits, int V, int chunk,
                                                                       const int32_t *__restrict__ hist, int64_t ld,
                                                                       const int32_t *__restrict__ step, int max_hist,
-                                                                      const TokenConstraintDesc *__restrict__ dp) {
+                                                                      const TokenConstraintDesc *__restrict__ dp,
+                                                                      float *__restrict__ pval, int32_t *__restrict__ pidx) {
     extern __shared__ uint32_t s_map[];
     __shared__ int32_t s_state;
+    __shared__ float s_bv[TC_THREADS / 64];
+    __shared__ int s_bi[TC_THREADS / 64];
     const int b = blockIdx.x, tid = threadIdx.x;
     const TokenConstraintDesc d = *dp;
     if (tid == 0) {
@@ -35,7 +38,13 @@
     }
     if (!logits) return;
     const int lo = blockIdx.y * chunk, hi = min(V, lo + chunk);
-    if (lo >= hi) return;
+    if (lo >= hi) {
+        if (pval && tid == 0) {
+            pval[b * gridDim.y + blockIdx.y] = -INFINITY;
+            pidx[b * gridDim.y + blockIdx.y] = 0x7fffffff;
+        }
+        return;
+    }
     const int wbase = lo >> 5, nw = ((hi - 1) >> 5) - wbase + 1;
     for (int w = tid; w <= nw; w += TC_THREADS) s_map[w] = 0u;
     __syncthreads();
@@ -54,6 +63,39 @@
 
     float *row = logits + (int64_t)b * V;
     const float ninf = -INFINITY;
+    if (pval) {
+        float bv = ninf;
+        int bi = 0x7fffffff;
+        for (int e = e0 + tid; e < e1; e += TC_THREADS) {
+            const int id = d.edge_tok[e];
+            if (id >= lo && id < hi) {
+                const float v = row[id];
+                if (v > bv || (v == bv && id < bi)) { bv = v; bi = id; }
+            }
+        }
+        if (d.completing[s])
+            for (int k = tid; k < d.n_end; k += TC_THREADS) {
+                const int id = d.end_ids[k];
+                if (id >= lo && id < hi) {
+                    const float v = row[id];
+                    if (v > bv || (v == bv && id < bi)) { bv = v; bi = id; }
+                }
+            }
+#pragma unroll
+        for (int o = 32; o > 0; o >>= 1) {
+            const float v = __shfl_xor(bv, o, 64);
+            const int i = __shfl_xor(bi, o, 64);
+            if (v > bv || (v == bv && i < bi)) { bv = v; bi = i; }
+        }
+        if ((tid & 63) == 0) { s_bv[tid >> 6] = bv; s_bi[tid >> 6] = bi; }
+        __syncthreads();
+        if (tid == 0) {
+            for (int w = 1; w < TC_THREADS / 64; ++w)
+                if (s_bv[w] > bv || (s_bv[w] == bv && s_bi[w] < bi)) { bv = s_bv[w]; bi = s_bi[w]; }
+            pval[b * gridDim.y + blockIdx.y] = bv;
+            pidx[b * gridDim.y + blockIdx.y] = bi;
+        }
+    }
     const int r0 = (int)(((16u - (unsigned)(reinterpret_cast<uintptr_t>(row) & 15u)) & 15u) >> 2);
     const int i0 = min(hi, lo + ((r0 - lo) & 3));
     const int n4 = (hi - i0) >> 2;
@@ -82,14 +124,18 @@
     }
 }
 
+int token_constraint_slices(int B) {
+    const int P = 256 / B;
+    return P < 1 ? 1 : (P > 8 ? 8 : P);
+}
+
 hipError_t launch_token_constraint(float *logits, int B, int V, const int32_t *hist, int64_t ld, const int32_t *step, int max_hist,
-                                   const TokenConstraintDesc *desc, hipStream_t s) {
-    if (V < 1 || V > TC_MAX_VOCAB || B < 1) return hipErrorInvalidValue;
-    int P = logits ? 256 / B : 1;
-    P = P < 1 ? 1 : (P > 8 ? 8 : P);
+                                   const TokenConstraintDesc *desc, hipStream_t s, float *pval, int32_t *pidx) {
+    if (V < 1 || V > TC_MAX_VOCAB || B < 1 || (pval && (!pidx || !logits))) return hipErrorInvalidValue;
+    const int P = logits ? token_constraint_slices(B) : 1;
     const int chunk = ((V + P - 1) / P + 31) & ~31;
     const size_t lds = logits ? (size_t)(chunk / 32 + 1) * sizeof(uint32_t) : 0;
-    hipLaunchKernelGGL(token_constraint_kernel, dim3(B, P), dim3(TC_THREADS), lds, s, logits, V, chunk, hist, ld, step, max_hist, desc);
+    hipLaunchKernelGGL(token_constraint_kernel, dim3(B, P), dim3(TC_THREADS), lds, s, logits, V, chunk, hist, ld, step, max_hist, desc, pval, pidx);
     return hipGetLastError();
 }
 
diff --git a/opus-pllm_amd/csrc/elementwise.hip b/opus-pllm_amd/csrc/elementwise.hip
--- a/opus-pllm_amd/csrc/elementwise.hip
+++ b/opus-pllm_amd/csrc/elementwise.hip
@@ -576,7 +576,7 @@
 }
 
 template <int LP>
-__device__ __forceinline__ void argmax_step_body(const float *__restrict__ pval, const int32_t *__restrict__ pidx,
+__device__ __forceinline__ void argmax_step_body(const float *__restrict__ pval, const int32_t *__restrict__ pidx, int nparts,
                                                  const int32_t *__restrict__ chosen, const int32_t *__restrict__ eos, int n_eos,
                                                  int pad_id, int32_t *__restrict__ finished, int32_t *__restrict__ out_ids,
                                                  int max_new, const int32_t *__restrict__ step, int32_t *__restrict__ next_tok,
@@ -585,8 +585,13 @@
                                                  const GenOutDesc *__restrict__ out, const float *__restrict__ lse_in = nullptr,
                                                  const float *__restrict__ raw_hist = nullptr) {
     const int b = blockIdx.x, lane = threadIdx.x;
-    float bv = pval[b * APART + lane];
-    int bi = pidx[b * APART + lane];
+    float bv = -INFINITY;
+    int bi = 0x7fffffff;
+    for (int j = lane; j < nparts; j += 64) {
+        const float v = pval[(int64_t)b * nparts + j];
+        const int i = pidx[(int64_t)b * nparts + j];
+        if (v > bv || (v == bv && i < bi)) { bv = v; bi = i; }
+    }
     const float mp = bv, sp = LP == 1 ? psum[b * APART + lane] : 0.f;
 #pragma unroll
     for (int o = 32; o > 0; o >>= 1) {
@@ -631,17 +636,17 @@
         if (!fin && st < max_new) atomicAdd(&n_unf[st], 1);
     }
 }
-__global__ __launch_bounds__(64) void argmax_step_kernel(const float *__restrict__ pval, const int32_t *__restrict__ pidx,
+__global__ __launch_bounds__(64) void argmax_step_kernel(const float *__restrict__ pval, const int32_t *__restrict__ pidx, int nparts,
                                                          const int32_t *__restrict__ chosen,
                                                          const int32_t *__restrict__ eos, int n_eos, int pad_id,
                                                          int32_t *__restrict__ finished, int32_t *__restrict__ out_ids,
                                                          int max_new, const int32_t *__restrict__ step,
                                                          int32_t *__restrict__ next_tok, int32_t *__restrict__ n_unf,
                                                          const int32_t *__restrict__ stop, int n_stop) {
-    argmax_step_body<0>(pval, pidx, chosen, eos, n_eos, pad_id, finished, out_ids, max_new, step, next_tok, n_unf, stop, n_stop,
+    argmax_step_body<0>(pval, pidx, nparts, chosen, eos, n_eos, pad_id, finished, out_ids, max_new, step, next_tok, n_unf, stop, n_stop,
                             nullptr, 0, nullptr, nullptr);
 }
-__global__ __launch_bounds__(64) void argmax_lse_step_kernel(const float *__restrict__ pval, const int32_t *__restrict__ pidx,
+__global__ __launch_bounds__(64) void argmax_lse_step_kernel(const float *__restrict__ pval, const int32_t *__restrict__ pidx, int nparts,
                                                              const int32_t *__restrict__ chosen,
                                                              const int32_t *__restrict__ eos, int n_eos, int pad_id,
                                                              int32_t *__restrict__ finished, int32_t *__restrict__ out_ids,
@@ -650,10 +655,10 @@
                                                              const int32_t *__restrict__ stop, int n_stop,
                                                              const float *__restrict__ logits, int V, const float *__restrict__ psum,
                                                              const GenOutDesc *__restrict__ out) {
-    argmax_step_body<1>(pval, pidx, chosen, eos, n_eos, pad_id, finished, out_ids, max_new, step, next_tok, n_unf, stop, n_stop,
+    argmax_step_body<1>(pval, pidx, nparts, chosen, eos, n_eos, pad_id, finished, out_ids, max_new, step, next_tok, n_unf, stop, n_stop,
                            logits, V, psum, out);
 }
-__global__ __launch_bounds__(64) void argmax_rawlp_step_kernel(const float *__restrict__ pval, const int32_t *__restrict__ pidx,
+__global__ __launch_bounds__(64) void argmax_rawlp_step_kernel(const float *__restrict__ pval, const int32_t *__restrict__ pidx, int nparts,
                                                                const int32_t *__restrict__ chosen,
                                                                const int32_t *__restrict__ eos, int n_eos, int pad_id,
                                                                int32_t *__restrict__ finished, int32_t *__restrict__ out_ids,
@@ -662,22 +667,22 @@
                                                                const int32_t *__restrict__ stop, int n_stop,
                                                                const float *__restrict__ logits, int V, const GenOutDesc *__restrict__ out,
                                                                const float *__restrict__ lse, const float *__restrict__ raw_hist) {
-    argmax_step_body<2>(pval, pidx, chosen, eos, n_eos, pad_id, finished, out_ids, max_new, step, next_tok, n_unf, stop, n_stop,
+    argmax_step_body<2>(pval, pidx, nparts, chosen, eos, n_eos, pad_id, finished, out_ids, max_new, step, next_tok, n_unf, stop, n_stop,
                         logits, V, nullptr, out, lse, raw_hist);
 }
-hipError_t launch_argmax_rawlp_step(const float *pval, const int32_t *pidx, const float *lse, const float *raw_hist,
+hipError_t launch_argmax_rawlp_step(const float *pval, const int32_t *pidx, int nparts, const float *lse, const float *raw_hist,
                                     const int32_t *chosen, int B, const int32_t *eos, int n_eos, int pad_id, int32_t *finished,
                                     int32_t *out_ids, int max_new, const int32_t *step, int32_t *next_tok, int32_t *n_unfinished,
                                     const int32_t *stop, int n_stop, const float *logits, int V, const GenOutDesc *out,
                                     hipStream_t s) {
-    hipLaunchKernelGGL(argmax_rawlp_step_kernel, dim3(B), dim3(64), 0, s, pval, pidx, chosen, eos, n_eos, pad_id, finished, out_ids,
+    hipLaunchKernelGGL(argmax_rawlp_step_kernel, dim3(B), dim3(64), 0, s, pval, pidx, nparts, chosen, eos, n_eos, pad_id, finished, out_ids,
                        max_new, step, next_tok, n_unfinished, stop, n_stop, logits, V, out, lse, raw_hist);
     return hipGetLastError();
 }
-hipError_t launch_argmax_step(const float *pval, const int32_t *pidx, const int32_t *chosen, int B, const int32_t *eos,
+hipError_t launch_argmax_step(const float *pval, const int32_t *pidx, int nparts, const int32_t *chosen, int B, const int32_t *eos,
                               int n_eos, int pad_id, int32_t *finished, int32_t *out_ids, int max_new, const int32_t *step,
                               int32_t *next_tok, int32_t *n_unfinished, const int32_t *stop, int n_stop, hipStream_t s) {
-    hipLaunchKernelGGL(argmax_step_kernel, dim3(B), dim3(64), 0, s, pval, pidx, chosen, eos, n_eos, pad_id, finished, out_ids,
+    hipLaunchKernelGGL(argmax_step_kernel, dim3(B), dim3(64), 0, s, pval, pidx, nparts, chosen, eos, n_eos, pad_id, finished, out_ids,
                        max_new, step, next_tok, n_unfinished, stop, n_stop);
     return hipGetLastError();
 }
@@ -685,11 +690,11 @@
     hipLaunchKernelGGL(argmax_lse_partial_kernel, dim3(APART, B), dim3(256), 0, s, logits, V, pval, pidx, psum);
     return hipGetLastError();
 }
-hipError_t launch_argmax_lse_step(const float *pval, const int32_t *pidx, const float *psum, const int32_t *chosen, int B,
+hipError_t launch_argmax_lse_step(const float *pval, const int32_t *pidx, int nparts, const float *psum, const int32_t *chosen, int B,
                                   const int32_t *eos, int n_eos, int pad_id, int32_t *finished, int32_t *out_ids, int max_new,
                                   const int32_t *step, int32_t *next_tok, int32_t *n_unfinished, const int32_t *stop, int n_stop,
                                   const float *logits, int V, const GenOutDesc *out, hipStream_t s) {
-    hipLaunchKernelGGL(argmax_lse_step_kernel, dim3(B), dim3(64), 0, s, pval, pidx, chosen, eos, n_eos, pad_id, finished, out_ids,
+    hipLaunchKernelGGL(argmax_lse_step_kernel, dim3(B), dim3(64), 0, s, pval, pidx, nparts, chosen, eos, n_eos, pad_id, finished, out_ids,
                        max_new, step, next_tok, n_unfinished, stop, n_stop, logits, V, psum, out);
     return hipGetLastError();
 }
diff --git a/opus-pllm_amd/csrc/gemm.hip b/opus-pllm_amd/csrc/gemm.hip
--- a/opus-pllm_amd/csrc/gemm.hip
+++ b/opus-pllm_amd/csrc/gemm.hip
@@ -2121,11 +2121,59 @@
                 store4<EPI>(p, m, panel * 16 + 4 * g, acc[i], up);
             }
         }
-    } else if (panel_ok) {
-#pragma unroll
-        for (int i = 0; i < MT; ++i) {
-            const int m = 16 * i + li;
-            if (m < p.M) store4<EPI>(p, m, panel * 16 + 4 * g, acc[i], acc[i]);
+    } else {
+        bool pick = false;
+        if constexpr (EPI == EPI_NONE) pick = p.amax_val != nullptr;
+        if (panel_ok && !(pick && p.amax_nostore)) {
+#pragma unroll
+            for (int i = 0; i < MT; ++i) {
+                const int m = 16 * i + li;
+                if (m < p.M) store4<EPI>(p, m, panel * 16 + 4 * g, acc[i], acc[i]);
+            }
+        }
+        if constexpr (EPI == EPI_NONE) {
+            if (pick) {
+                float *pv = reinterpret_cast<float *>(smem);
+                int *pi = reinterpret_cast<int *>(smem + 8 * MP * 4);
+                __syncthreads();
+                const int nb = panel * 16 + 4 * g;
+#pragma unroll
+                for (int i = 0; i < MT; ++i) {
+                    float bv = -INFINITY;
+                    int bi = 0x7fffffff;
+#pragma unroll
+                    for (int r = 0; r < 4; ++r) {
+                        if (panel_ok && nb + r < p.N) {
+                            float v = acc[i][r];
+                            if (p.bias) v += p.bias[nb + r];
+                            if (v > bv || (v == bv && nb + r < bi)) { bv = v; bi = nb + r; }
+                        }
+                    }
+#pragma unroll
+                    for (int o = 16; o < 64; o <<= 1) {
+                        const float v = __shfl_xor(bv, o, 64);
+                        const int ix = __shfl_xor(bi, o, 64);
+                        if (v > bv || (v == bv && ix < bi)) { bv = v; bi = ix; }
+                    }
+                    if (g == 0) {
+                        pv[wave * MP + 16 * i + li] = bv;
+                        pi[wave * MP + 16 * i + li] = bi;
+                    }
+                }
+                __syncthreads();
+                if (tid < MP && tid < p.M) {
+                    float bv = pv[tid];
+                    int bi = pi[tid];
+#pragma unroll
+                    for (int w = 1; w < 8; ++w) {
+                        const float v = pv[w * MP + tid];
+                        const int ix = pi[w * MP + tid];
+                        if (v > bv || (v == bv && ix < bi)) { bv = v; bi = ix; }
+                    }
+                    p.amax_val[(int64_t)tid * p.amax_ld + blockIdx.x] = bv;
+                    p.amax_idx[(int64_t)tid * p.amax_ld + blockIdx.x] = bi;
+                }
+            }
         }
     }
 }
@@ -2137,7 +2185,7 @@
     }
     const int blocks = cdiv((p.N + 15) >> 4, 8), chunks = p.K / 64;
     int ks = 1;
-    if (p.ws && blocks < 200) {
+    if (p.ws && blocks < 200 && !p.wide_whole_k) {
         ks = 256 / blocks;
         ks = ks > 8 ? 8 : ks;
         if (ks > chunks / 8) ks = chunks / 8;
@@ -2150,9 +2198,12 @@
     if (ea != hipSuccess) return ea;
     gemm_plan_set(p, KC_WIDE, MT, 0, 0, 0, 0, ks, ks == 1 ? GC_NONE : GC_SLABS);
     if (W8 && p.ran_w8) *p.ran_w8 = 1;
-    if (ks > 1 && p.row_ssq) {
+    const bool pick = EPI == EPI_NONE && p.amax_val && p.amax_idx && ks == 1 && p.out_f32 && !p.residual && p.amax_ld >= blocks;
+    if (pick && p.amax_done) *p.amax_done = 1;
+    if ((ks > 1 && p.row_ssq) || (p.amax_val && !pick)) {
         GemmParams q = p;
-        q.row_ssq = nullptr;
+        if (ks > 1) q.row_ssq = nullptr;
+        if (!pick) { q.amax_val = nullptr; q.amax_nostore = 0; }
         OPUS_LAUNCH(KC_WIDE, (gemm_wide_kernel<MT, EPI, W8>), dim3(blocks, ks), dim3(512), lds, s, q, ks);
     } else {
         OPUS_LAUNCH(KC_WIDE, (gemm_wide_kernel<MT, EPI, W8>), dim3(blocks, ks), dim3(512), lds, s, p, ks);
@@ -2312,8 +2363,8 @@
     if (klass) *klass = skinny ? KC_SKINNY : KC_TILE;
     if (p.Af && !skinny && !mid) return hipErrorInvalidValue;
     if (p.Af && p.epi == EPI_GELU) return hipErrorInvalidValue;
-    const bool to_stream = mid && !p.Af && p.N < 16384 && gemm_stream_ok(p);
-    const bool to_wide = !to_stream && mid && !p.Af && !mid_v1 && (p.N >= 16384 || p.force_wide || narrow_wide());
+    const bool to_stream = mid && !p.Af && p.N < 16384 && !p.wide_whole_k && gemm_stream_ok(p);
+    const bool to_wide = !to_stream && mid && !p.Af && !mid_v1 && (p.N >= 16384 || p.force_wide || p.wide_whole_k || narrow_wide());
     if (p.a_tiled && !to_stream) return hipErrorInvalidValue;
     if (p.c_tiled && (p.out_f32 || !(to_stream || to_wide) || ((p.epi == EPI_SILU_GU16 ? p.N / 2 : p.N) & 63))) return hipErrorInvalidValue;
     if (p.row_ssq && skinny) return hipErrorInvalidValue;
@@ -2330,9 +2381,9 @@
             case EPI_GELU: return launch_skinny_e<EPI_GELU, false>(p, s);
             case EPI_SILU_GU16: return launch_skinny_e<EPI_SILU_GU16, false>(p, s);
         }
-    } else if (mid && !p.Af && !mid_v1 && p.N < 16384 && gemm_stream_ok(p)) {
+    } else if (to_stream && !mid_v1) {
         return launch_gemm_stream(p, s);
-    } else if (mid && !p.Af && !mid_v1 && (p.N >= 16384 || p.force_wide || narrow_wide())) {
+    } else if (to_wide) {
         const bool m2 = p.M <= 32;
         switch (p.epi) {
             case EPI_NONE: return m2 ? launch_wide<2, EPI_NONE>(p, s) : launch_wide<4, EPI_NONE>(p, s);
diff --git a/opus-pllm_amd/eval_ddp.py b/opus-pllm_amd/eval_ddp.py
--- a/opus-pllm_amd/eval_ddp.py
+++ b/opus-pllm_amd/eval_ddp.py
@@ -63,6 +63,8 @@
             extra["guidance_scale"] = float(guidance_scale)
         if logprobs_out is not None:
             extra.update(return_dict_in_generate=True, output_token_logprobs=True)
+        if logits_out is not None and hasattr(m, "keep_last_logits"):
+            m.keep_last_logits(True)
         with torch.inference_mode():
             out = m.generate(ids, [q["input"] for q in batch], attention_mask=mask, pad_token_id=tokenizer.eos_token_id,
                              do_sample=temperature > 0, temperature=temperature, top_p=top_p,
diff --git a/opus-pllm_amd/model.py b/opus-pllm_amd/model.py
--- a/opus-pllm_amd/model.py
+++ b/opus-pllm_amd/model.py
@@ -1388,6 +1388,9 @@
             raise KeyError(name)
         return v
 
+    def keep_last_logits(self, on: bool = True) -> None:
+        _cabi.check(self._lib.opus_keep_last_logits(self._ctx, 1 if on else 0))
+
     def last_logits(self, B: int) -> torch.Tensor:
         s = self._enter()
         with torch.cuda.stream(self._stream):
```

Measured after the change: 259.7 proteins/s (median of 3 runs). About the same (-0.0%).
